# nihofm/volren

Measured on AMD Instinct MI355X. Metric: Msamples/s (pixels x spp / s), volume path tracing, higher is better.
Workload: dtype f32; 1 GPU; BASELINE configs[1] 'c2': smoke.brick, no transfer function, 1024x1024, 1024 spp, seed 42, fov 40; parallelism=1 GPU, 1 fused launch(es)/frame (sample pool budget 64 GiB)

## Files before the change

volren_amd/csrc/capi.cpp:

```cpp
#include "../../include/volren_amd.h"

#include <algorithm>
#include <climits>
#include <cmath>
#include <cstring>
#include <filesystem>
#include <functional>
#include <iostream>
#include <stdexcept>
#include <memory>
#include <string>
#include <vector>

#include "imageio.h"
#include "renderer.h"
#include "sharded.h"
#include "vr_device.h"
#include "vr_math_probe.h"

struct vr_renderer {
    vr::RendererHIP impl;
    int device = 0;
};

struct vr_sharded {
    std::vector<vr_renderer*> parts;
    std::unique_ptr<vr::ShardedRenderer> impl;
    std::string transport, collective;
};

static thread_local std::string g_last_error;

static int guard(const std::function<void()>& fn) {
    try {
        fn();
        g_last_error.clear();
        return VR_OK;
    } catch (const std::exception& e) {
        g_last_error = e.what();
        return VR_ERR;
    } catch (...) {
        g_last_error = "unknown error";
        return VR_ERR;
    }
}
static int fail(int code, const char* msg) { g_last_error = msg; return code; }
#define NEED(r) do { if (!(r)) return fail(VR_ERR_ARG, "null renderer"); } while (0)
#define NEED_SHARDED(s) do { if (!(s)) return fail(VR_ERR_ARG, "null sharded renderer"); } while (0)
#define NEED_DEVICE() do { if (vr_device_count() <= 0) return fail(VR_ERR_NO_DEVICE, "no HIP device available (libvolren_amd has no CPU path)"); } while (0)

static void use_device(vr_renderer* r) { VR_HIP(hipSetDevice(r->device)); }

static int read_back(vr_renderer* r, float* out, void (vr::RendererHIP::*download)(float*)) {
    NEED(r);
    if (!out) return fail(VR_ERR_ARG, "null argument");
    NEED_DEVICE();
    return guard([&] { use_device(r); (r->impl.*download)(out); });
}

namespace {
using Rn = vr::RendererHIP;
struct IntParam {
    const char* name;
    int (*get)(Rn&);
    void (*set)(Rn&, int);
    int lo, hi;
    const char* refusal;
};
vr::SceneParams next_launch(Rn& R) { vr::SceneParams P; R.fill_params(P); return P; }
vr::PathtraceKernel next_kernel(Rn& R) { return vr::pathtrace_kernel_of(next_launch(R), R.tuning.wide_addressing != 0, R.tuning.stats != nullptr); }
void set_grid_frame(Rn& R, int v) {
    if (!R.volume || v < 0 || (size_t)v >= R.volume->n_grid_frames()) throw std::runtime_error("grid_frame_counter out of range");
    R.volume->grid_frame_counter = (size_t)v;
}
#define VR_GET(expr) [](Rn& R) -> int { return expr; }
#define VR_SET(stmt) [](Rn& R, int v) { stmt; }
#define VR_INT(field) VR_GET(R.field), VR_SET(R.field = v)
#define VR_FLAG(field) VR_GET(R.field ? 1 : 0), VR_SET(R.field = v != 0)
#define VR_ANY 1, 0, nullptr
#define VR_READ_ONLY(expr) VR_GET(expr), nullptr, VR_ANY
const IntParam kIntParams[] = {
    { "sample", VR_GET(R.sample), VR_SET(R.sample = v; R.drop_tile_samples()), VR_ANY },
    { "sppx", VR_INT(sppx), VR_ANY },
    { "seed", VR_INT(seed), VR_ANY },
    { "bounces", VR_INT(bounces), VR_ANY },
    { "show_environment", VR_FLAG(show_environment), VR_ANY },
    { "tonemapping", VR_FLAG(tonemapping), VR_ANY },
    { "integrator", VR_INT(integrator), VR_ANY },
    { "fast_math", VR_FLAG(fast_math), VR_ANY },
    { "variance", VR_INT(variance), 0, 1, "variance: 0 (off) or 1 (keep the per-pixel second moments)" },
    { "denoise_iterations", VR_INT(denoise_iterations), 0, vr::kDenoiseMaxIterations, "denoise_iterations must be in [0, 10]" },
    { "denoise_moments", VR_GET(R.denoise_moments), VR_SET(R.set_denoise_moments(v)), VR_ANY },
    { "denoise_resolve", VR_GET(R.denoise_resolve), VR_SET(R.set_denoise_resolve(v)), VR_ANY },
    { "denoise_layers", VR_GET(R.denoise_layers), VR_SET(R.set_denoise_layers(v)), VR_ANY },
    { "denoise_filter", VR_GET(R.denoise_filter), VR_SET(R.set_denoise_filter(v)), VR_ANY },
    { "coalesce_trace", VR_GET(R.coalesce_trace ? 1 : 0), VR_SET(R.flush_pending(); R.coalesce_trace = v != 0), VR_ANY },
    { "majorant_layout", VR_INT(majorant_layout), -1, 1, "majorant_layout: -1 (per grid, chosen at commit), 0 (linear), 1 (4x4x4-cell blocks)" },
    { "majorant_blocked", VR_READ_ONLY(next_launch(R).density.maj_blocked) },
    { "kernel_variant", VR_READ_ONLY(next_kernel(R).variant) },
    { "kernel_variant_reason", VR_READ_ONLY(next_kernel(R).reason) },
    { "tf_float_atlas", VR_FLAG(tf_float_atlas), VR_ANY },
    { "wide_addressing", VR_INT(tuning.wide_addressing), 0, 1, "wide_addressing: 0 (by the tables' sizes), 1 (always the kernels with 64-bit gather addresses)" },
    { "kernel_wide", VR_READ_ONLY(next_kernel(R).wide ? 1 : 0) },
    { "env_div_safe", VR_READ_ONLY(R.environment && R.environment->cdf_div_safe ? 1 : 0) },
    { "env_compact", VR_READ_ONLY(R.environment && R.environment->envmap_rgbe ? 1 : 0) },
    { "pending_samples", VR_READ_ONLY(R.pending_samples()) },
    { "gpu_encoder", VR_FLAG(gpu_encoder), VR_ANY },
    { "sample_pool_mb", VR_GET((int)(R.sample_pool_bytes >> 20)), VR_SET(R.sample_pool_bytes = (size_t)v << 20), 16, 65536,
      "sample_pool_mb must be in [16, 65536] (item indices of a sub-launch are 32-bit: < 2^32 RGBA32F items)" },
    { "seed_table_mb", VR_GET(R.seed_table_budget_mb()), VR_SET(R.seed_table_mb = v), -1, Rn::kSeedTableMaxMb,
      "seed_table_mb must be in [0, 8192] (0 = no table), or -1 for the default min(4096, sample_pool_mb / 4)" },
    { "seed_table_max_samples", VR_INT(seed_table_max_samples), 0, INT_MAX, "seed_table_max_samples must be >= 0 (0 = as many as seed_table_mb holds)" },
    { "seed_table_samples", VR_READ_ONLY(R.seed_table_samples()) },
    { "seed_table_fills", VR_READ_ONLY(R.seed_table_fills()) },
    { "launch_target_ms", VR_INT(launch_target_ms), 0, INT_MAX, "launch_target_ms must be >= 0 (0 = no sizing by time)" },
    { "expected_skip", VR_INT(expected_skip), 0, 1, "expected_skip: 0 (march every step) or 1 (drop the steps of empty space by the clear-distance table)" },
    { "expected_stats", VR_INT(expected_stats), 0, 1, "expected_stats: 0 (off) or 1 (the expected-value passes count their work)" },
    { "order_tiles", VR_INT(order_tiles), 0, 2, "order_tiles: 0 (never), 1 (tile subsets), 2 (always)" },
    { "sky_tiles", VR_INT(sky_tiles), 0, 1, "sky_tiles: 0 (every tile through the path tracer) or 1 (tiles whose camera rays cannot hit the volume's box are rendered apart)" },
    { "last_sky_tiles", VR_READ_ONLY(R.last_sky_tiles) },
    { "grid_frame_counter", VR_GET(R.volume ? (int)R.volume->grid_frame_counter : 0), set_grid_frame, VR_ANY },
    { "n_grid_frames", VR_READ_ONLY(R.volume ? (int)R.volume->n_grid_frames() : 0) },
    { "last_launches", VR_READ_ONLY(R.last_launches) },
    { "adaptive_rounds", VR_READ_ONLY(R.adaptive_rounds) },
    { "width", VR_READ_ONLY(R.resolution.x) },
    { "height", VR_READ_ONLY(R.resolution.y) },
};
#undef VR_GET
#undef VR_SET
#undef VR_INT
#undef VR_FLAG
#undef VR_ANY
#undef VR_READ_ONLY
const IntParam& int_param(const char* name, bool writable) {
    for (const IntParam& p : kIntParams)
        if (!strcmp(p.name, name) && (p.set || !writable)) return p;
    throw std::runtime_error(std::string("unknown int parameter: ") + name);
}

struct FloatField { float* ptr; int count; void (*check)(const float* values, int count) = nullptr; };
FloatField float_field(vr::RendererHIP& R, const std::string& n) {
    if (n == "tonemap_exposure") return { &R.tonemap_exposure, 1 };
    if (n == "tonemap_gamma") return { &R.tonemap_gamma, 1 };
    if (n == "albedo") return { &R.albedo.x, 3 };
    if (n == "phase") return { &R.phase, 1 };
    if (n == "density_scale") return { &R.density_scale, 1 };
    if (n == "emission_scale") return { &R.emission_scale, 1 };
    if (n == "vol_clip_min") return { &R.vol_clip_min.x, 3 };
    if (n == "vol_clip_max") return { &R.vol_clip_max.x, 3 };
    if (n == "cam_pos") return { &R.camera.pos.x, 3 };
    if (n == "cam_dir") return { &R.camera.dir.x, 3 };
    if (n == "cam_up") return { &R.camera.up.x, 3 };
    if (n == "cam_fov") return { &R.camera.fov_degree, 1 };
    if (n == "env_strength") { if (!R.environment) throw std::runtime_error("no environment"); return { &R.environment->strength, 1 }; }
    if (n == "env_transform") { if (!R.environment) throw std::runtime_error("no environment"); return { R.environment->transform.m, 9 }; }
    if (n == "tf_window_left") { if (!R.transferfunc) throw std::runtime_error("no transfer function"); return { &R.transferfunc->window_left, 1 }; }
    if (n == "tf_window_width") { if (!R.transferfunc) throw std::runtime_error("no transfer function"); return { &R.transferfunc->window_width, 1 }; }
    if (n == "volume_transform") { if (!R.volume) throw std::runtime_error("no volume"); return { R.volume->transform.m, 16 }; }
    if (n == "denoise_sigma") return { R.denoise_sigma, 5, [](const float* values, int count) {
        if (count != 5) throw std::runtime_error("denoise_sigma takes 5 values (colour, normal, depth, coverage, albedo)");
        for (int i = 0; i < 5; ++i)
            if (!(values[i] >= vr::kDenoiseSigmaMin && values[i] <= vr::kDenoiseSigmaMax))
                throw std::runtime_error("denoise_sigma: every value must be in [2^-60, 2^60]");
    } };
    if (n == "denoise_alpha") return { &R.denoise_alpha, 1, [](const float* values, int count) {
        if (count == 1 && !(values[0] >= vr::kTemporalAlphaMin && values[0] <= vr::kTemporalAlphaMax)) throw std::runtime_error("denoise_alpha must be in [2^-20, 1]");
    } };
    if (n == "denoise_reject") return { &R.denoise_reject, 1, [](const float* values, int count) {
        if (count == 1 && !(values[0] == 0.0f || (values[0] >= vr::kTemporalRejectMin && values[0] <= vr::kTemporalRejectMax)))
            throw std::runtime_error("denoise_reject must be 0 (off) or in [2^-10, 2^20]");
    } };
    if (n == "denoise_ridge") return { &R.denoise_ridge, 1, [](const float* values, int count) {
        if (count == 1 && !vr::regress_ridge_ok(values[0])) throw std::runtime_error("denoise_ridge must be 0 (zero order) or in [2^-20, 2^20]");
    } };
    throw std::runtime_error("unknown float parameter: " + n);
}
}

extern "C" {

const char* vr_last_error(void) { return g_last_error.c_str(); }
const char* vr_version(void) { return "volren_amd 0.1 (gfx950)"; }

int vr_device_count(void) {
    int n = 0;
    if (hipGetDeviceCount(&n) != hipSuccess) return 0;
    return n;
}

int vr_create(vr_renderer** out, int device, int width, int height) {
    if (!out) return fail(VR_ERR_ARG, "null out pointer");
    *out = nullptr;
    NEED_DEVICE();
    vr_renderer* r = nullptr;
    const int rc = guard([&] {
        if (width <= 0 || height <= 0) throw std::runtime_error("vr_create: resolution must be positive");
        r = new vr_renderer();
        r->device = device;
        use_device(r);
        r->impl.resolution = { width, height };
        r->impl.init();
    });
    if (rc != VR_OK) { delete r; return rc; }
    *out = r;
    return VR_OK;
}

void vr_destroy(vr_renderer* r) {
    if (!r) return;
    (void)hipSetDevice(r->device);
    delete r;
}

int vr_resize(vr_renderer* r, int w, int h) {
    NEED(r);
    return guard([&] { use_device(r); if (w <= 0 || h <= 0) throw std::runtime_error("vr_resize: resolution must be positive"); r->impl.resize((uint32_t)w, (uint32_t)h); r->impl.sample = 0; });
}

int vr_load_volume(vr_renderer* r, const char* path) {
    NEED(r);
    if (!path) return fail(VR_ERR_ARG, "null path");
    return guard([&] {
        use_device(r);
        std::cout << "load volume: " << path << std::endl;
        if (std::filesystem::is_directory(path)) r->impl.volume = vr::Volume::load_folder(path);
        else r->impl.volume = std::make_shared<vr::Volume>(std::string(path));
        r->impl.density_scale = 1.f;
        r->impl.scale_and_move_to_unit_cube();
        r->impl.commit();
        r->impl.sample = 0;
    });
}

int vr_set_volume_path(vr_renderer* r, const char* path) {
    NEED(r);
    if (!path) return fail(VR_ERR_ARG, "null path");
    return guard([&] {
        if (std::filesystem::is_directory(path)) r->impl.volume = vr::Volume::load_folder(path);
        else r->impl.volume = std::make_shared<vr::Volume>(std::string(path));
    });
}

int vr_volume_aabb(vr_renderer* r, const char* name, float out[6]) {
    NEED(r);
    if (!out) return fail(VR_ERR_ARG, "null output");
    return guard([&] {
        if (!r->impl.volume || r->impl.volume->grids.empty()) throw std::runtime_error("vr_volume_aabb: no volume");
        const auto bb = r->impl.volume->AABB(name ? name : "density");
        out[0] = bb.first.x; out[1] = bb.first.y; out[2] = bb.first.z; out[3] = bb.second.x; out[4] = bb.second.y; out[5] = bb.second.z;
    });
}
int vr_volume_minorant_majorant(vr_renderer* r, const char* name, float out[2]) {
    NEED(r);
    if (!out) return fail(VR_ERR_ARG, "null output");
    return guard([&] {
        if (!r->impl.volume || r->impl.volume->grids.empty()) throw std::runtime_error("vr_volume_minorant_majorant: no volume");
        const auto mm = r->impl.volume->minorant_majorant(name ? name : "density");
        out[0] = mm.first; out[1] = mm.second;
    });
}

int vr_load_envmap(vr_renderer* r, const char* path) {
    NEED(r);
    if (!path) return fail(VR_ERR_ARG, "null path");
    return guard([&] { use_device(r); r->impl.environment = std::make_shared<vr::Environment>(std::string(path)); r->impl.sample = 0; });
}

int vr_load_transferfunc(vr_renderer* r, const char* path) {
    NEED(r);
    if (!path) return fail(VR_ERR_ARG, "null path");
    return guard([&] {
        use_device(r);
        r->impl.transferfunc = std::make_shared<vr::TransferFunction>(std::string(path));
// ... 619 lines not shown
```

volren_amd/csrc/renderer.cpp:

```cpp
#include "renderer.h"

#include <algorithm>
#include <cfloat>
#include <cmath>
#include <cstdlib>
#include <cstring>
#include <iostream>
#include <mutex>

#include "vr_adaptive.h"
#include "vr_device.h"
#include "vr_math.h"
#include "vr_path_probe.h"
#include "vr_probe.h"
#include "vr_sky_tiles.h"
#include "vr_upsample.h"

namespace vr {

mat3 Camera::view_inverse() const {
    const vec3 f = normalize(dir);
    const vec3 s = normalize(cross(f, up));
    const vec3 u = cross(s, f);
    mat3 r(0.0f);
    r.m[0] = s.x; r.m[1] = s.y; r.m[2] = s.z;
    r.m[3] = u.x; r.m[4] = u.y; r.m[5] = u.z;
    r.m[6] = -f.x; r.m[7] = -f.y; r.m[8] = -f.z;
    return r;
}

RendererHIP::~RendererHIP() {
    if (ev0_) (void)hipEventDestroy(ev0_);
    if (ev1_) (void)hipEventDestroy(ev1_);
    for (hipEvent_t e : pt_events_) (void)hipEventDestroy(e);
    if (seed_event_) (void)hipEventDestroy(seed_event_);
}

void RendererHIP::init() {
    int n_dev = 0;
    if (hipGetDeviceCount(&n_dev) != hipSuccess || n_dev == 0)
        throw std::runtime_error("RendererHIP::init: no HIP device available (this renderer has no CPU path)");
    if (!volume) volume = std::make_shared<Volume>();
    if (!environment) {
        const float white[3] = { 1.f, 1.f, 1.f };
        environment = std::make_shared<Environment>(white, 1, 1);
    }
    if (!ev0_) { VR_HIP(hipEventCreate(&ev0_)); VR_HIP(hipEventCreate(&ev1_)); }
    if (!status_) {
        status_ = make_device_buffer(16 * sizeof(uint32_t));
        VR_HIP(hipMemset(status_->get(), 0, 16 * sizeof(uint32_t)));
    }
    if (!color && resolution.x > 0 && resolution.y > 0) resize((uint32_t)resolution.x, (uint32_t)resolution.y);
}

void RendererHIP::resize(uint32_t w, uint32_t h) {
    if (w == 0 || h == 0) throw std::runtime_error("RendererHIP::resize: empty framebuffer");
    pending_n_ = 0; pending_ = LaunchInputs{};
    resolution = { (int)w, (int)h };
    color = make_device_buffer((size_t)w * h * 4 * sizeof(float));
    display.reset();
    sized_ = Sized{};
    drop_tile_samples();
    drop_seed_table();
    VR_HIP(hipMemset(color->get(), 0, color->size_bytes()));
    if (!tiles_host_.empty()) set_tiles(tiles_host_);
}

void RendererHIP::reset() { sample = 0; drop_tile_samples(); }

static void check_grid_bytes(size_t bytes, const char* what, const int32_t nb[3]);
constexpr size_t kBlockedMajorantBricks = (size_t)1 << 18;
static size_t brick_records(const BrickGridHIP& g);

void RendererHIP::commit() {
    flush_pending();
    rate_samples_per_ms_ = 0.0; rate_pending_samples_ = 0.0;
    density_grids.clear();
    emission_grids.clear();
    majorant_emission = 0.f;
    maj_key_ = MajKey{};
    std::cout << "Preparing brick grids for HIP..." << std::endl;
    std::vector<size_t> with_emission;
    for (const auto& frame : volume->grids) {
        Volume::GridPtr density_grid = frame.at("density");
        density_grids.push_back(grid_to_device(density_grid));
        Volume::GridPtr emission_grid;
        for (const char* name : { "flame", "flames", "temperature" }) {
            auto it = frame.find(name);
            if (it != frame.end()) { emission_grid = it->second; break; }
        }
        if (emission_grid) {
            emission_grids.push_back(grid_to_device(emission_grid));
            majorant_emission = std::max(majorant_emission, emission_grid->minorant_majorant().second);
            if (emission_grids.size() == density_grids.size()) with_emission.push_back(density_grids.size() - 1);
        }
    }
    for (size_t f : with_emission) {
        BrickGridHIP& gd = density_grids[f];
        BrickGridHIP& ge = emission_grids[f];
        if (!(VR_BRICK_HEADERS && gd.atlas && ge.atlas && grids_can_pair(gd, ge))) continue;
        try {
            const size_t n_rec = brick_records(gd);
            check_grid_bytes(n_rec * kPairBlockBytes, "the paired density + emission atlas", gd.nb);
            auto paired = make_device_buffer(n_rec * kPairBlockBytes);
            launch_pair_atlas(gd.atlas->as<uint8_t>(), ge.atlas->as<uint8_t>(), paired->as<uint8_t>(), n_rec, stream);
            VR_HIP(hipGetLastError());
            VR_HIP(hipStreamSynchronize(stream));
            gd.atlas_paired = ge.atlas_paired = paired;
            gd.maj_blocked = gd.n_active > kBlockedMajorantBricks;
        } catch (const std::exception& e) {
            (void)hipGetLastError();
            std::cerr << "volren_amd: no room for the paired density + emission atlas of frame " << f << " (" << e.what() << "): the run-time kernel variant serves it" << std::endl;
        }
    }
}

BrickGridHIP RendererHIP::grid_to_device(const Volume::GridPtr& grid) {
    if (auto f16 = std::dynamic_pointer_cast<DenseGridF16>(grid)) return dense_grid_to_device(f16);
    if (gpu_encoder)
        if (auto dense = std::dynamic_pointer_cast<DenseGrid>(grid)) return dense_to_bricks_on_device(dense);
    return brick_grid_to_device(Volume::to_brick_grid(grid));
}

static void check_grid_bytes(size_t bytes, const char* what, const int32_t nb[3]) {
    size_t free_b = 0, total_b = 0;
    if (hipMemGetInfo(&free_b, &total_b) != hipSuccess) { (void)hipGetLastError(); return; }
    const size_t reserve = (size_t)1 << 30;
    if (bytes + reserve > free_b)
        throw std::runtime_error(std::string("grid upload: ") + what + " of a grid of " + std::to_string(nb[0]) + " x " + std::to_string(nb[1]) + " x " + std::to_string(nb[2]) +
                                 " bricks needs " + std::to_string(bytes >> 20) + " MiB of device memory, " + std::to_string(free_b >> 20) + " MiB are free");
}
static void set_layout(BrickGridHIP& out) {
    for (int i = 0; i < 3; ++i) out.mshift[i] = std::max(3, ceil_log2((uint32_t)out.nb[i]));
    if (out.mshift[0] + out.mshift[1] + out.mshift[2] > 30 || (uint64_t)out.nb[0] * out.nb[1] * out.nb[2] > 400000000ull)
        throw std::runtime_error("grid upload: more than 4e8 bricks");
    if ((uint64_t)out.nb[1] * out.nb[2] >= (1ull << 24) || out.nb[0] >= (1 << 24))
        throw std::runtime_error("grid upload: brick counts beyond the 24-bit index arithmetic of the kernels (n_bricks.y * n_bricks.z < 2^24)");
    const size_t cells = majorant_table_cells((uint32_t)(out.mshift[0] + out.mshift[1] + out.mshift[2]));
    out.majorant = make_device_buffer(cells * sizeof(float));
    out.majorant16 = make_device_buffer(cells * sizeof(uint16_t));
}
static size_t brick_records(const BrickGridHIP& g) { return (size_t)g.nb[0] * g.nb[1] * g.nb[2]; }

static void upload_range_words(BrickGridHIP& out, const uvec3 nb, const Buf3D<uint32_t>& range, const std::vector<Buf3D<uint32_t>>& mips) {
    if (mips.size() > 3) throw std::runtime_error("grid upload: at most 3 range mips are supported");
    std::vector<uint32_t> words(range.data);
    out.n_mips = (int)mips.size();
    for (int m = 0; m <= 3; ++m) out.mip_off[m] = 0;
    for (int m = 1; m <= out.n_mips; ++m) {
        const auto& mm = mips[m - 1];
        const uint32_t rnd = (1u << m) - 1u;
        if (mm.stride.x != ((nb.x + rnd) >> m) || mm.stride.y != ((nb.y + rnd) >> m) || mm.stride.z != ((nb.z + rnd) >> m))
            throw std::runtime_error("grid upload: range mip dimensions are not ceil(n_bricks / 2^m)");
        out.mip_off[m] = (int32_t)words.size();
        words.insert(words.end(), mm.data.begin(), mm.data.end());
    }
    out.n_cells = (int32_t)words.size();
    out.range_words = make_device_buffer(words.size() * sizeof(uint32_t));
    out.range_words->upload(words.data(), words.size() * sizeof(uint32_t));
    set_layout(out);
}

BrickGridHIP RendererHIP::dense_to_bricks_on_device(const std::shared_ptr<DenseGrid>& g) {
    BrickGridHIP out;
    auto up8 = [](uint32_t v) { return ((v + 7u) / 8u + 7u) / 8u * 8u; };
    const int32_t dim[3] = { (int32_t)g->dim.x, (int32_t)g->dim.y, (int32_t)g->dim.z };
    const int32_t nb[3] = { (int32_t)up8(g->dim.x), (int32_t)up8(g->dim.y), (int32_t)up8(g->dim.z) };
    const size_t n = (size_t)nb[0] * nb[1] * nb[2];
    for (int i = 0; i < 3; ++i) out.nb[i] = nb[i];
    out.transform = g->transform;
    DeviceBuffer dense(g->voxels.size() * sizeof(float)), flag(n * sizeof(uint32_t));
    dense.upload(g->voxels.data(), g->voxels.size() * sizeof(float), stream);
    int32_t mdim[4][3];
    size_t total = 0;
    out.n_mips = 3;
    for (int m = 0; m <= 3; ++m) {
        for (int i = 0; i < 3; ++i) mdim[m][i] = (nb[i] + (1 << m) - 1) >> m;
        out.mip_off[m] = (int32_t)total;
        total += (size_t)mdim[m][0] * mdim[m][1] * mdim[m][2];
    }
    out.n_cells = (int32_t)total;
    out.range_words = make_device_buffer(total * sizeof(uint32_t));
    set_layout(out);
    uint32_t* words = out.range_words->as<uint32_t>();
    launch_encode_ranges(dense.as<float>(), dim, nb, words, flag.as<uint32_t>(), stream);
    VR_HIP(hipGetLastError());
    check_grid_bytes(brick_records(out) * (kBrickBlockBytes + sizeof(BrickRec) + 8), "the brick-linear atlas", out.nb);
    out.atlas = make_device_buffer(brick_records(out) * kBrickBlockBytes);
    VR_HIP(hipMemsetAsync(out.atlas->get(), 0, out.atlas->size_bytes(), stream));
    out.bricks = make_device_buffer(brick_records(out) * sizeof(BrickRec));
    VR_HIP(hipMemsetAsync(out.bricks->get(), 0, out.bricks->size_bytes(), stream));
    out.rng = make_device_buffer(brick_records(out) * 2 * sizeof(float));
    VR_HIP(hipMemsetAsync(out.rng->get(), 0, out.rng->size_bytes(), stream));
    launch_encode_bricks(dense.as<float>(), dim, nb, words, flag.as<uint32_t>(), out.bricks->as<BrickRec>(), out.rng->as<float>(), out.atlas->as<uint8_t>(), stream);
    for (int m = 1; m <= 3; ++m) launch_range_mip(words + out.mip_off[m - 1], mdim[m - 1], words + out.mip_off[m], mdim[m], stream);
    VR_HIP(hipGetLastError());
    VR_HIP(hipStreamSynchronize(stream));
    {
        std::vector<uint32_t> flags(n);
        flag.download(flags.data(), n * sizeof(uint32_t), stream);
        for (uint32_t f : flags) out.n_active += f != 0u;
    }
    return out;
}

constexpr uint64_t kFnv1aStart = 1469598103934665603ull;
static uint64_t fnv1a(const void* p, size_t n, uint64_t h = kFnv1aStart) {
    const uint8_t* b = static_cast<const uint8_t*>(p);
    for (size_t i = 0; i < n; ++i) { h ^= b[i]; h *= 1099511628211ull; }
    return h;
}
void RendererHIP::grid_checksums(const BrickGridHIP& g, uint64_t out[3]) const {
    const DeviceBufferPtr bufs[3] = { g.bricks, g.atlas, g.range_words };
    for (int i = 0; i < 3; ++i) {
        out[i] = 0;
        if (!bufs[i]) continue;
        std::vector<uint8_t> h(bufs[i]->size_bytes());
        bufs[i]->download(h.data(), h.size(), stream);
        out[i] = fnv1a(h.data(), h.size());
    }
}

BrickGridHIP RendererHIP::dense_grid_to_device(const std::shared_ptr<DenseGridF16>& g) {
    BrickGridHIP out;
    const uvec3 nb = g->range.stride;
    out.nb[0] = (int)nb.x; out.nb[1] = (int)nb.y; out.nb[2] = (int)nb.z;
    out.dim[0] = (int)g->dim.x; out.dim[1] = (int)g->dim.y; out.dim[2] = (int)g->dim.z;
    if (g->dim.x > 65535u || g->dim.y > 65535u || g->dim.z > 65535u) throw std::runtime_error("dense_grid_to_device: more than 65535 voxels along an axis");
    out.transform = g->transform;
    const uint32_t bx = (g->dim.x + 3u) / 4u, by = (g->dim.y + 3u) / 4u, bz = (g->dim.z + 3u) / 4u;
    if ((uint64_t)bx * by * bz > (1ull << 31)) throw std::runtime_error("dense_grid_to_device: more than 2^31 blocks");
    out.dblk[0] = (int)bx; out.dblk[1] = (int)by;
    std::vector<uint16_t> blocked((size_t)bx * by * bz * 64u, 0);
    for (uint32_t z = 0; z < g->dim.z; ++z)
        for (uint32_t y = 0; y < g->dim.y; ++y) {
            const uint16_t* row = &g->voxels[((size_t)z * g->dim.y + y) * g->dim.x];
            for (uint32_t x = 0; x < g->dim.x; ++x) blocked[dense_blocked_index(x, y, z, bx, by)] = row[x];
        }
// ... 74 lines not shown
    v.bricks = g.bricks ? g.bricks->as<BrickRec>() : nullptr;
    v.atlas = paired ? g.atlas_paired->as<uint8_t>() : (g.atlas ? g.atlas->as<uint8_t>() : nullptr);
    v.dense = g.dense ? g.dense->as<uint16_t>() : nullptr;
    for (int i = 0; i < 3; ++i) v.dim[i] = g.dim[i];
    for (int i = 0; i < 2; ++i) v.dblk[i] = g.dblk[i];
    v.majorant = g.majorant->as<float>();
    v.majorant16 = g.majorant16->as<uint16_t>();
    v.rng = g.rng ? g.rng->as<float>() : nullptr;
    v.atlas_f32 = g.atlas_f32 ? g.atlas_f32->as<float>() : nullptr;
    for (int i = 0; i < 3; ++i) v.nb[i] = g.nb[i];
    for (int i = 0; i < 3; ++i) { v.mshift[i] = g.mshift[i]; v.mlim[i] = (float)(8u << g.mshift[i]); }
    v.n_mips = g.n_mips;
    v.maj_blocked = maj_blocked ? 1 : 0;
    v.maj_outside = (int32_t)majorant_padded_cells((uint32_t)(g.mshift[0] + g.mshift[1] + g.mshift[2]));
    return v;
}

void RendererHIP::fill_params(SceneParams& P) {
    if (!volume || volume->grids.empty() || density_grids.empty())
        throw std::runtime_error("RendererHIP::trace: no volume committed");
    if (volume->grid_frame_counter >= density_grids.size())
        throw std::runtime_error("RendererHIP::trace: grid_frame_counter out of range (commit() after changing the volume)");
    memset(&P, 0, sizeof P);
    Uniforms& u = P.u;
    u.bounces = bounces;
    u.seed = seed;
    u.show_environment = show_environment ? 1 : 0;
    u.integrator = integrator;
    P.env_div_safe = environment->cdf_div_safe ? 1 : 0;
    copy3(u.cam_pos, camera.pos);
    u.cam_fov = camera.fov_degree;
    const mat3 ct = camera.view_inverse();
    memcpy(u.cam_transform, ct.m, sizeof ct.m);
    P.cam_z = camera_z(camera.fov_degree);
    const auto [bb_min, bb_max] = volume->AABB();
    const auto [mn, maj] = volume->minorant_majorant();
    copy3(u.vol_bb_min, bb_min + vol_clip_min * (bb_max - bb_min));
    copy3(u.vol_bb_max, bb_min + vol_clip_max * (bb_max - bb_min));
    u.vol_minorant = mn * density_scale;
    u.vol_majorant = maj * density_scale;
    u.vol_inv_majorant = 1.f / (maj * density_scale);
    copy3(u.vol_albedo, albedo);
    u.vol_phase_g = phase;
    u.vol_density_scale = density_scale;
    u.vol_emission_scale = emission_scale;
    u.vol_emission_norm = majorant_emission > 0.f ? 1.f / std::fmax(majorant_emission, 1e-4f) : 1.f;
    const BrickGridHIP& density = density_grids[volume->grid_frame_counter];
    const mat4 dt = volume->transform * density.transform;
    const mat4 dti = inverse(dt);
    memcpy(u.vol_density_transform, dt.m, sizeof dt.m);
    memcpy(u.vol_density_inv_transform, dti.m, sizeof dti.m);
    P.density = make_view(density);
    if (volume->grid_frame_counter < emission_grids.size()) {
        const BrickGridHIP& emission = emission_grids[volume->grid_frame_counter];
        const mat4 et = volume->transform * emission.transform;
        const mat4 eti = inverse(et);
        memcpy(u.vol_emission_transform, et.m, sizeof et.m);
        memcpy(u.vol_emission_inv_transform, eti.m, sizeof eti.m);
        const mat4 efd = eti * dt;
        memcpy(P.emission_from_density, efd.m, sizeof efd.m);
        P.paired = (density.atlas_paired && density.atlas_paired == emission.atlas_paired && pathtrace_scene_reasons(P) == 0) ? 1 : 0;
        if (P.paired) P.density = make_view(density, true, majorant_layout < 0 ? density.maj_blocked : majorant_layout == 1);
        P.emission = make_view(emission, P.paired != 0);
        u.has_emission = 1;
    }
    if (transferfunc) {
        u.use_tf = 1;
        u.tf_size = transferfunc->size();
        u.tf_window_left = transferfunc->window_left;
        u.tf_window_width = transferfunc->window_width;
        P.tf_lut = transferfunc->lut_ssbo->as<float>();
    }
    const mat3 eit = inverse(environment->transform);
    memcpy(u.env_transform, environment->transform.m, sizeof eit.m);
    memcpy(u.env_inv_transform, eit.m, sizeof eit.m);
    u.env_strength = environment->strength;
    u.env_imp_inv_dim[0] = u.env_imp_inv_dim[1] = 1.f / (float)environment->dimension();
    u.env_imp_base_mip = (int)std::floor(std::log2((float)environment->dimension()));
    P.envmap = environment->envmap->as<float>();
    P.env_rgbe = environment->envmap_rgbe ? environment->envmap_rgbe->as<uint32_t>() : nullptr;
    P.env_w = environment->width; P.env_h = environment->height;
    P.env_avg_w = environment->avg_importance; P.env_avg_w_set = 1;
    P.impmap = environment->impmap->as<float>();
    P.imp_dim = (int)environment->dimension();
    P.env_cdf = environment->cdf->as<float>();
    u.resolution[0] = resolution.x; u.resolution[1] = resolution.y;
}

void RendererHIP::update_majorants(const LaunchInputs& in, BrickGridHIP& g) {
    if (in.maj == maj_key_) return;
    launch_majorants(in.P, g.range_words->as<uint32_t>(), g.nb, g.mip_off, g.n_mips, g.mshift, g.majorant->as<float>(), g.majorant16->as<uint16_t>(), in.stream);
    VR_HIP(hipGetLastError());
    maj_key_ = in.maj;
}

void RendererHIP::set_tiles(const std::vector<int32_t>& tile_ids) {
    flush_pending();
    tiles_host_ = tile_ids;
    tiles_dev_.reset();
    if (tile_ids.empty()) return;
    if (resolution.x > 0) {
        const int n_all = tile_count(resolution.x, resolution.y);
        for (int32_t t : tile_ids)
            if (t < 0 || t >= n_all) throw std::runtime_error("set_tiles: tile id out of range");
    }
    tiles_dev_ = make_device_buffer(tile_ids.size() * sizeof(int32_t));
    tiles_dev_->upload(tile_ids.data(), tile_ids.size() * sizeof(int32_t));
}

std::vector<int32_t> RendererHIP::costliest_first(const SceneParams& P, const std::vector<int32_t>& tile_ids, int n_tiles) const {
    const Uniforms& u = P.u;
    const int W = u.resolution[0], H = u.resolution[1], tiles_x = vr::tiles_x(W);
    std::vector<int32_t> ids(tile_ids);
    if (ids.empty()) { ids.resize((size_t)n_tiles); for (int i = 0; i < n_tiles; ++i) ids[(size_t)i] = i; }
    auto chord = [&](float px, float py) {
        float d[3] = { (px - 0.5f * (float)W) / (float)H, (py - 0.5f * (float)H) / (float)H, P.cam_z };
        float w[3];
        for (int i = 0; i < 3; ++i) w[i] = u.cam_transform[i] * d[0] + u.cam_transform[3 + i] * d[1] + u.cam_transform[6 + i] * d[2];
        const float len = std::sqrt(w[0] * w[0] + w[1] * w[1] + w[2] * w[2]);
        float t0 = 0.f, t1 = FLT_MAX;
        for (int i = 0; i < 3; ++i) {
            const float inv = 1.f / (w[i] / len);
            const float a = (u.vol_bb_min[i] - u.cam_pos[i]) * inv, b = (u.vol_bb_max[i] - u.cam_pos[i]) * inv;
            t0 = std::fmax(t0, std::fmin(a, b)); t1 = std::fmin(t1, std::fmax(a, b));
        }
        return t1 > t0 ? t1 - t0 : 0.f;
    };
    std::vector<float> cost(ids.size());
    for (size_t k = 0; k < ids.size(); ++k) {
        const float x0 = (float)((ids[k] % tiles_x) * 16), y0 = (float)((ids[k] / tiles_x) * 16);
        const float x1 = std::fmin(x0 + 16.f, (float)W), y1 = std::fmin(y0 + 16.f, (float)H);
        cost[k] = std::fmax(std::fmax(std::fmax(chord(x0, y0), chord(x1, y0)), std::fmax(chord(x0, y1), chord(x1, y1))), chord(0.5f * (x0 + x1), 0.5f * (y0 + y1)));
    }
    std::vector<int32_t> perm(ids.size());
    for (size_t k = 0; k < perm.size(); ++k) perm[k] = (int32_t)k;
    const size_t seg = (ids.size() + 7) / 8;
    for (size_t b = 0; b < ids.size(); b += seg)
        std::stable_sort(perm.begin() + (ptrdiff_t)b, perm.begin() + (ptrdiff_t)std::min(ids.size(), b + seg), [&](int32_t x, int32_t y) { return cost[(size_t)x] > cost[(size_t)y]; });
    std::vector<int32_t> ordered(ids.size());
    for (size_t k = 0; k < ids.size(); ++k) ordered[k] = ids[(size_t)perm[k]];
    return ordered;
}

uint64_t RendererHIP::tile_order_key(const SceneParams& P, const std::vector<int32_t>& ids, int n_tiles) const {
    const Uniforms& u = P.u;
    uint64_t key = kFnv1aStart;
    auto mix = [&key](const void* p, size_t nbytes) { key = fnv1a(p, nbytes, key); };
    mix(u.cam_pos, sizeof u.cam_pos); mix(u.cam_transform, sizeof u.cam_transform); mix(&P.cam_z, sizeof P.cam_z);
    mix(u.vol_bb_min, sizeof u.vol_bb_min); mix(u.vol_bb_max, sizeof u.vol_bb_max); mix(u.resolution, sizeof u.resolution); mix(&n_tiles, sizeof n_tiles);
    if (!ids.empty()) mix(ids.data(), ids.size() * sizeof(int32_t));
    return key ? key : 1;
}

RendererHIP::SplitTiles RendererHIP::split_tiles(const SceneParams& P, const std::vector<int32_t>& ids, int n_tiles, bool ordered) {
    const int tag = ordered ? 2 : 1;
    uint64_t key = fnv1a(&tag, sizeof tag, tile_order_key(P, ids, n_tiles));
    key = key ? key : 1;
    if (split_key_ != key) {
        std::vector<int32_t> march, sky;
        sky_split_tiles(P, ids, n_tiles, march, sky);
        if (!sky.empty()) {
            if (ordered && !march.empty()) march = costliest_first(P, march, (int)march.size());
            march.insert(march.end(), sky.begin(), sky.end());
            ensure_buffer(split_dev_, march.size() * sizeof(int32_t));
            split_dev_->upload(march.data(), march.size() * sizeof(int32_t), stream);
        }
        split_n_sky_ = (int)sky.size();
        split_key_ = key;
    }
    SplitTiles s;
    if (split_n_sky_ > 0) {
        s.n_sky = split_n_sky_;
        s.n_march = n_tiles - split_n_sky_;
        s.march = split_dev_->as<int32_t>();
        s.sky = s.march + s.n_march;
    }
    return s;
}

const int32_t* RendererHIP::tile_order(const SceneParams& P, const std::vector<int32_t>& ids, int n_tiles) {
    const uint64_t key = tile_order_key(P, ids, n_tiles);
    if (order_dev_ && order_key_ == key && order_dev_->size_bytes() == (size_t)n_tiles * sizeof(int32_t)) return order_dev_->as<int32_t>();
    const std::vector<int32_t> ordered = costliest_first(P, ids, n_tiles);
    ensure_buffer(order_dev_, ordered.size() * sizeof(int32_t));
    order_dev_->upload(ordered.data(), ordered.size() * sizeof(int32_t), stream);
    order_key_ = key;
    return order_dev_->as<int32_t>();
}

bool RendererHIP::LaunchInputs::same_launch_as(const LaunchInputs& o) const {
    return memcmp(&P, &o.P, sizeof P) == 0 && frame == o.frame && maj == o.maj && tuning == o.tuning && order_tiles == o.order_tiles && launch_target_ms == o.launch_target_ms &&
           fast_math == o.fast_math && variance == o.variance && sky_tiles == o.sky_tiles && sample_pool_bytes == o.sample_pool_bytes && stream == o.stream;
}

void RendererHIP::capture(LaunchInputs& in) {
    if (!color) throw std::runtime_error("RendererHIP::trace: no framebuffer (call resize first)");
    if (integrator == 2 && !transferfunc) throw std::runtime_error("RendererHIP::trace: integrator 2 (direct volume rendering) needs a transfer function");
    if (integrator < 0 || integrator > 3) throw std::runtime_error("RendererHIP::trace: unknown integrator");
    if (fast_math && transferfunc) throw std::runtime_error("RendererHIP::trace: fast_math is not available while a transfer function is bound (it misses the 1e-3 bound there); set fast_math 0");
    if (!volume || volume->grids.empty() || density_grids.empty()) throw std::runtime_error("RendererHIP::trace: no volume committed");
    if (volume->grid_frame_counter >= density_grids.size()) throw std::runtime_error("RendererHIP::trace: grid_frame_counter out of range (commit() after changing the volume)");
    {
        BrickGridHIP& g = density_grids[volume->grid_frame_counter];
        const bool build = transferfunc && tf_float_atlas && !g.dense && g.atlas && g.rng && !g.atlas_f32 && !g.atlas_f32_failed;
        const bool drop = (!transferfunc || !tf_float_atlas) && (g.atlas_f32 || g.atlas_f32_failed);
        if (build || drop) flush_pending();
        if (build) {
            try {
                const size_t n_blocks = g.atlas->size_bytes() / kBrickBlockBytes, want = n_blocks * 512u * sizeof(float);
                auto drop_others = [&] { for (BrickGridHIP& other : density_grids) if (&other != &g) other.atlas_f32.reset(); };
                size_t free_b = 0, total_b = 0;
                if (hipMemGetInfo(&free_b, &total_b) != hipSuccess) { (void)hipGetLastError(); free_b = ~(size_t)0; }
                if (want > free_b / 2) drop_others();
                try { g.atlas_f32 = make_device_buffer(want); }
                catch (const std::exception&) { (void)hipGetLastError(); drop_others(); g.atlas_f32 = make_device_buffer(want); }
                launch_decode_atlas(g.rng->as<float>(), g.atlas->as<uint8_t>(), g.atlas_f32->as<float>(), n_blocks, stream);
                VR_HIP(hipGetLastError());
            } catch (const std::exception& e) {
                (void)hipGetLastError();
                g.atlas_f32.reset();
                g.atlas_f32_failed = true;
                std::cerr << "volren_amd: no room for the decoded float atlas (" << (g.atlas->size_bytes() / kBrickBlockBytes * 2048u >> 20) << " MiB): transfer-function taps read the byte atlas (" << e.what() << ")" << std::endl;
            }
        }
        if (drop) { g.atlas_f32.reset(); g.atlas_f32_failed = false; }
    }
    fill_params(in.P);
    in.frame = volume->grid_frame_counter;
    in.maj = MajKey{};
    in.maj.density_scale = density_scale;
    in.maj.tf_version = transferfunc ? transferfunc->version : 0;
    in.maj.wl = transferfunc ? transferfunc->window_left : 0.f;
    in.maj.ww = transferfunc ? transferfunc->window_width : 0.f;
    in.maj.frame = in.frame;
    in.maj.blocked = in.P.density.maj_blocked;
    in.tuning = tuning;
    in.order_tiles = order_tiles; in.launch_target_ms = launch_target_ms; in.fast_math = fast_math ? 1 : 0; in.variance = variance != 0 ? 1 : 0; in.sky_tiles = sky_tiles != 0 ? 1 : 0;
    in.sample_pool_bytes = sample_pool_bytes;
    in.stream = stream;
    in.env = environment; in.tf = transferfunc;
    in.keep[0] = environment->envmap; in.keep[1] = environment->impmap; in.keep[2] = environment->cdf;
    in.keep[3] = transferfunc ? transferfunc->lut_ssbo : DeviceBufferPtr();
    in.keep[4] = environment->envmap_rgbe;
}

int RendererHIP::samples_per_launch(const LaunchInputs& in, int n_tiles) const {
    const size_t per_sample = pathtrace_pool_floats(in.tuning, n_tiles, 1) * sizeof(float);
    int per_launch = (int)std::max<size_t>(1, in.sample_pool_bytes / per_sample);
    const size_t lim = (size_t)0xFFFFFFFFu / ((size_t)n_tiles * 256u);
    per_launch = (int)std::min<size_t>((size_t)per_launch, lim > 8 ? lim - 8 : 1);
    if (per_launch > 32) per_launch -= per_launch % 32;
    return per_launch;
}

void RendererHIP::submit_tile_set(const LaunchInputs& in, int first, int n) {
    if (n <= 0) return;
    const int n_tiles = tile_set_size();
    const bool ordered = in.order_tiles >= 2 || (in.order_tiles == 1 && tiles_dev_);
    const SplitTiles split = in.splits_sky() ? split_tiles(in.P, tiles_dev_ ? tiles_host_ : std::vector<int32_t>(), n_tiles, ordered) : SplitTiles{};
    if (split.n_sky > 0) {
        const int per_launch = prepare_submit(in, first, n, split.n_march, split.n_sky);
        open_timing_window(in.stream);
        submit(in, first, n, split.march, split.n_march, per_launch, split.sky, split.n_sky);
        close_timing_window(in.stream);
        return;
    }
    const int32_t* tiles = ordered ? tile_order(in.P, tiles_host_, n_tiles) : (tiles_dev_ ? tiles_dev_->as<int32_t>() : nullptr);
    const int per_launch = prepare_submit(in, first, n, n_tiles);
    open_timing_window(in.stream);
    submit(in, first, n, tiles, n_tiles, per_launch);
    close_timing_window(in.stream);
}

int RendererHIP::tile_set_size() const { return tiles_dev_ ? (int)tiles_host_.size() : tile_count(resolution.x, resolution.y); }

void RendererHIP::open_timing_window(hipStream_t s) { VR_HIP(hipEventRecord(ev0_, s)); last_launches = 0; pt_events_used_ = 0; }
void RendererHIP::close_timing_window(hipStream_t s) { VR_HIP(hipEventRecord(ev1_, s)); timing_pending_ = true; }

int RendererHIP::prepare_submit(const LaunchInputs& in, int first, int n, int n_tiles, int n_sky) {
    if (n <= 0) return 0;
    hipStream_t stream = in.stream;
    update_majorants(in, density_grids.at(in.frame));
    int per_launch = n_tiles > 0 ? std::min(samples_per_launch(in, n_tiles + n_sky), n) : n;
    for (; n_tiles > 0;) {
        const size_t need = pathtrace_pool_floats(in.tuning, n_tiles, per_launch) * sizeof(float);
        if (pool_ && pool_->size_bytes() >= need) break;
        if (pool_) { VR_HIP(hipStreamSynchronize(stream)); pool_.reset(); }
        try { pool_ = make_device_buffer(need); break; }
        catch (const std::exception&) {
            (void)hipGetLastError();
            if (per_launch <= 1) throw;
            per_launch = std::max(1, per_launch / 2);
            if (per_launch > 32) per_launch -= per_launch % 32;
        }
    }
    if (!workspace_ && n_tiles > 0) {
        workspace_ = make_device_buffer(pathtrace_workspace_floats() * sizeof(float));
        if (const char* e = std::getenv("VR_TEST_POISON_WORKSPACE"); e && *e == '1') VR_HIP(hipMemsetAsync(workspace_->get(), 0xFF, workspace_->size_bytes(), stream));
    }
    if (const char* e = std::getenv("VR_TEST_POISON_WORKSPACE"); e && *e == '2' && n_tiles > 0) {
        VR_HIP(hipMemsetAsync(workspace_->get(), 0xFF, workspace_->size_bytes(), stream));
        VR_HIP(hipMemsetAsync(pool_->get(), 0xFF, pool_->size_bytes(), stream));
    }
    if (in.launch_target_ms > 0 && in.kernel().item_integrator == 0) harvest_rate(false);
    if (in.variance && ensure_buffer(sized_.moments, color->size_bytes())) {
        VR_HIP(hipMemsetAsync(sized_.moments->get(), 0, color->size_bytes(), stream));
        if (first > 0) sized_.moments_n = -1;
    }
    sized_.moments_n = !in.variance ? -1 : (first == 0 ? n : (sized_.moments_n == first ? first + n : -1));
    return per_launch;
}

void RendererHIP::submit(const LaunchInputs& in, int first, int n, const int32_t* tiles, int n_tiles, int per_launch, const int32_t* sky, int n_sky) {
    const SceneParams& P = in.P;
    last_sky_tiles = n_sky;
    hipStream_t stream = in.stream;
    const PathtraceKernel kernel = in.kernel();
    const bool pt_kernel = kernel.item_integrator == 0;
    const double px_samples = (double)(n_tiles + n_sky) * 256.0;
    const uint64_t key = [&] {
        uint64_t h = kFnv1aStart;
        auto mix = [&h](const void* p, size_t nbytes) { h = fnv1a(p, nbytes, h); };
        const Uniforms& u = P.u;
        mix(&u.bounces, sizeof u.bounces); mix(u.vol_albedo, sizeof u.vol_albedo); mix(&u.vol_phase_g, sizeof u.vol_phase_g); mix(&u.vol_density_scale, sizeof u.vol_density_scale);
        mix(&u.use_tf, sizeof u.use_tf); mix(&u.tf_window_left, sizeof u.tf_window_left); mix(&u.tf_window_width, sizeof u.tf_window_width); mix(&u.integrator, sizeof u.integrator);
        mix(&u.has_emission, sizeof u.has_emission); mix(u.resolution, sizeof u.resolution); mix(u.vol_bb_min, sizeof u.vol_bb_min); mix(u.vol_bb_max, sizeof u.vol_bb_max);
        const size_t frame = in.frame; mix(&frame, sizeof frame); mix(&n_tiles, sizeof n_tiles);
        const uint64_t tfv = in.maj.tf_version; mix(&tfv, sizeof tfv);
        return h ? h : 1ull;
    }();
    auto cap_by_rate = [&](int planned) {
        if (in.launch_target_ms <= 0 || rate_samples_per_ms_ <= 0.0) return planned;
        const double cap = rate_samples_per_ms_ * (double)in.launch_target_ms / px_samples;
        int c = cap >= (double)planned ? planned : std::max(1, (int)cap);
        if (c > 32) c -= c % 32;
        return c;
    };
    int probe = 0;
    if (pt_kernel && in.launch_target_ms > 0) {
        const bool known = rate_samples_per_ms_ > 0.0 && rate_key_ == key;
        if (!known && px_samples * (double)std::min(per_launch, n) > (double)(1u << 26)) {
            rate_samples_per_ms_ = 0.0;
            probe = (int)std::min<double>(32.0, std::max(1.0, (double)(1u << 24) / px_samples));
            probe = std::min(probe, n);
        } else per_launch = cap_by_rate(per_launch);
    }
    float* moments = in.variance ? sized_.moments->as<float>() : nullptr;
    for (int done = 0; done < n;) {
        if (n_tiles > 0) ++last_launches;
        const int m = probe > 0 ? probe : std::min(per_launch, n - done);
        hipEvent_t eb = nullptr, ee = nullptr;
        if (pt_kernel) {
            while (pt_events_.size() < pt_events_used_ + 2) { hipEvent_t e; VR_HIP(hipEventCreate(&e)); pt_events_.push_back(e); }
            eb = pt_events_[pt_events_used_]; ee = pt_events_[pt_events_used_ + 1];
            pt_events_used_ += 2;
        }
        int seed_samples = 0;
        const uint32_t* seed_table = kernel.reads_seed_table ? seed_table_for(P, first + done, m, stream, &seed_samples) : nullptr;
        launch_pathtrace(in.tuning, P, color->as<float>(), n_tiles > 0 ? pool_->as<float>() : nullptr, n_tiles > 0 ? workspace_->as<float>() : nullptr, status_->as<uint32_t>() + 1, tiles, n_tiles, first + 1 + done, m,
                         status_->as<uint32_t>(), stream, in.fast_math != 0, eb, ee, moments, seed_table, seed_samples, sky, n_sky);
        VR_HIP(hipGetLastError());
        done += m;
        if (pt_kernel) { rate_pending_samples_ = px_samples * (double)m; rate_pending_key_ = key; }
        if (probe > 0) {
            probe = 0;
            harvest_rate(true);
            per_launch = cap_by_rate(per_launch);
        }
    }
}

int RendererHIP::seed_table_samples_for(long long mb, int w, int h) {
    if (mb <= 0 || w <= 0 || h <= 0) return 0;
    const long long per_sample = (long long)tile_count(w, h) * 256 * (long long)sizeof(uint32_t);
    return (int)std::min<long long>((mb << 20) / per_sample, 1 << 24);
}

void RendererHIP::drop_seed_table() {
    seed_table_.reset();
    seed_cap_ = seed_filled_ = 0;
    seed_failed_ = false;
}

const uint32_t* RendererHIP::seed_table_for(const SceneParams& P, int s0, int n, hipStream_t stream, int* samples) {
    *samples = 0;
    const int W = P.u.resolution[0], H = P.u.resolution[1], budget_mb = seed_table_budget_mb();
    if (seed_key_[0] != P.u.seed || seed_key_[1] != W || seed_key_[2] != H || seed_budget_mb_ != budget_mb || seed_max_samples_ != seed_table_max_samples) {
        drop_seed_table();
        seed_key_[0] = P.u.seed; seed_key_[1] = W; seed_key_[2] = H; seed_budget_mb_ = budget_mb; seed_max_samples_ = seed_table_max_samples;
    }
    int max_samples = seed_table_samples_for(budget_mb, W, H);
    if (seed_table_max_samples > 0) max_samples = std::min(max_samples, seed_table_max_samples);
    if (max_samples <= 0 || (seed_failed_ && !seed_table_) || s0 < 0 || n <= 0) return nullptr;
    const size_t per_sample = (size_t)tile_count(W, H) * 256u * sizeof(uint32_t);
    const int want = (int)std::min<long long>((long long)s0 + n, max_samples);
    if (!seed_event_) VR_HIP(hipEventCreateWithFlags(&seed_event_, hipEventDisableTiming));
    if (seed_table_ && seed_filled_ > 0 && stream != seed_stream_) { VR_HIP(hipStreamWaitEvent(stream, seed_event_, 0)); seed_stream_ = stream; }
    if (want > seed_cap_ && !seed_failed_) {
        const int cap = (int)std::min<long long>(max_samples, std::max<long long>(want, 2ll * seed_cap_));
        DeviceBufferPtr grown;
        try { grown = make_device_buffer((size_t)cap * per_sample); }
        catch (const std::exception& e) {
            (void)hipGetLastError();
            seed_failed_ = true;
            static std::once_flag once;
            std::call_once(once, [&] { fprintf(stderr, "volren_amd: note: no memory for the path-seed table (%zu MiB: %s); new paths hash their seeds (slower; results unchanged)\n", ((size_t)cap * per_sample) >> 20, e.what()); });
            if (!seed_table_) return nullptr;
        }
        if (grown) {
            if (const char* e = std::getenv("VR_TEST_POISON_WORKSPACE"); e && *e == '2') VR_HIP(hipMemsetAsync(grown->get(), 0xFF, grown->size_bytes(), stream));
            if (seed_filled_ > 0) VR_HIP(hipMemcpyAsync(grown->get(), seed_table_->get(), (size_t)seed_filled_ * per_sample, hipMemcpyDeviceToDevice, stream));
            if (seed_table_) VR_HIP(hipStreamSynchronize(stream));
            seed_table_ = grown;
            seed_cap_ = cap;
        }
    }
    const int upto = std::min(want, seed_cap_);
    if (upto > seed_filled_) {
        launch_seed_fill(seed_table_->as<uint32_t>(), (uint32_t)P.u.seed, W, H, seed_filled_, upto, stream);
        VR_HIP(hipGetLastError());
        VR_HIP(hipEventRecord(seed_event_, stream));
        seed_stream_ = stream;
        seed_filled_ = upto;
        ++seed_fills_;
    }
    *samples = seed_filled_;
    return seed_filled_ > 0 ? seed_table_->as<uint32_t>() : nullptr;
}

void RendererHIP::harvest_rate(bool wait) {
    if (rate_pending_samples_ <= 0.0 || pt_events_used_ < 2) return;
    hipEvent_t eb = pt_events_[pt_events_used_ - 2], ee = pt_events_[pt_events_used_ - 1];
    if (wait) VR_HIP(hipEventSynchronize(ee));
    else if (hipEventQuery(ee) != hipSuccess) { (void)hipGetLastError(); return; }
    float ms = 0.f;
    if (hipEventElapsedTime(&ms, eb, ee) != hipSuccess || !(ms > 0.f)) { (void)hipGetLastError(); return; }
    rate_samples_per_ms_ = rate_pending_samples_ / (double)ms;
    rate_key_ = rate_pending_key_;
    rate_pending_samples_ = 0.0;
}

void RendererHIP::trace() {
    if (ragged())
        throw std::runtime_error("trace: the frame holds per-tile sample counts of render_adaptive (a ragged frame): reset(), or continue with render_adaptive");
    if (!coalesce_trace) { flush_pending(); LaunchInputs in; capture(in); submit_tile_set(in, sample, 1); sample += 1; return; }
    LaunchInputs now;
    capture(now);
    if (pending_n_ > 0 && (sample != pending_first_ + pending_n_ || !now.same_launch_as(pending_))) flush_pending();
    if (pending_n_ == 0) {
        pending_ = std::move(now);
        pending_first_ = sample;
        pending_cap_ = samples_per_launch(pending_, tile_set_size());
    }
    ++pending_n_;
    ++sample;
    if (pending_n_ >= pending_cap_) flush_pending();
}

void RendererHIP::flush_pending() {
    if (pending_n_ <= 0) return;
    const int n = pending_n_, first = pending_first_;
    pending_n_ = 0;
    LaunchInputs in = std::move(pending_);
    pending_ = LaunchInputs{};
    submit_tile_set(in, first, n);
}

void RendererHIP::render(int n) {
    flush_pending();
    if (ragged()) throw std::runtime_error("render: the frame holds per-tile sample counts of render_adaptive (a ragged frame): reset(), or continue with render_adaptive");
    if (n <= 0) n = sppx - sample;
    if (n <= 0) return;
    LaunchInputs in;
    capture(in);
    submit_tile_set(in, sample, n);
    sample += n;
}

void RendererHIP::draw() {
    flush_pending();
    if (!color) return;
    draw_from(*color);
}

void RendererHIP::draw_from(const DeviceBuffer& src) {
    ensure_buffer(display, src.size_bytes());
    VR_HIP(hipMemcpyAsync(display->get(), src.get(), src.size_bytes(), hipMemcpyDeviceToDevice, stream));
    if (tonemapping) {
        launch_tonemap(display->as<float>(), (int32_t)(src.size_bytes() / (4 * sizeof(float))), 1, tonemap_exposure, tonemap_gamma, stream);
        VR_HIP(hipGetLastError());
    }
}

double RendererHIP::last_kernel_ms() {
    flush_pending();
    if (timing_pending_) {
        VR_HIP(hipEventSynchronize(ev1_));
        float ms = 0.f;
        VR_HIP(hipEventElapsedTime(&ms, ev0_, ev1_));
        last_ms_ = (double)ms;
        last_pathtrace_ms_ = 0.0;
        for (size_t i = 0; i + 1 < pt_events_used_; i += 2)
            if (hipEventElapsedTime(&ms, pt_events_[i], pt_events_[i + 1]) == hipSuccess) last_pathtrace_ms_ += (double)ms;
        (void)hipGetLastError();
        timing_pending_ = false;
    }
    return last_ms_;
}

double RendererHIP::last_pathtrace_ms() { (void)last_kernel_ms(); return last_pathtrace_ms_; }

void RendererHIP::sched_stats(bool enable, unsigned long long out[32]) {
    flush_pending();
// ... 443 lines not shown
        throw std::runtime_error(me + "the expected-value pass ran with rays = " + std::to_string(sized_.rays) + "; rays >= 2 is needed (one ray gives the coverage of the pixel's centre, not of its area)");
    if ((size_t)resolution.x * (size_t)resolution.y * 2u > (size_t)INT32_MAX) throw std::runtime_error(me + "frame too large (32-bit pixel indices)");
}

void RendererHIP::run_resolve() {
    LaunchInputs in;
    capture(in);
    const size_t bytes = (size_t)resolution.x * resolution.y * 4 * sizeof(float);
    ensure_buffer(sized_.rs_bg, bytes); ensure_buffer(sized_.rs_part, bytes); ensure_buffer(sized_.resolved, bytes);
    launch_resolve(in.P, color->as<float>(), sized_.features->as<float>(), sized_.rays, sized_.rs_bg->as<float>(), sized_.rs_part->as<float>(), sized_.resolved->as<float>(), stream);
    VR_HIP(hipGetLastError());
}

void RendererHIP::resolve() {
    flush_pending();
    check_resolve("resolve: ", false);
    run_resolve();
}

void RendererHIP::download_resolved(float* rgba) { download_whole(sized_.resolved, rgba, "resolved: no resolve since the last resize (call resolve first)"); }

void RendererHIP::download_resolve_background(float* rgba) {
    download_whole(sized_.resolved ? sized_.rs_bg : nullptr, rgba, "resolve_background: no resolve since the last resize (call resolve first)");
}

void RendererHIP::download_denoised_layer(float* rgba) {
    download_whole(sized_.layer_valid ? sized_.layer : nullptr, rgba, "denoised_layer: no denoise with denoise_layers = 1 since the last resize");
}

void RendererHIP::upsample(int factor, int rays) {
    if (factor < kUpsampleMinFactor || factor > kUpsampleMaxFactor) throw std::runtime_error("upsample: factor must be 2..4");
    if (rays < 1 || rays > kExpectedMaxRays) throw std::runtime_error("upsample: rays must be 1.." + std::to_string(kExpectedMaxRays));
    flush_pending();
    if (!sized_.layer_valid) throw std::runtime_error("upsample: no denoise with denoise_layers = 1 since the last resize (its layer is what the call upsamples)");
    if (!sized_.layer_guided)
        throw std::runtime_error("upsample: the last denoise ran with denoise_layers = 0 and its guide has replaced the layer's (denoise with denoise_layers = 1 again; denoised_layer stays readable)");
    if (!tiles_host_.empty() && !sized_.layer_gathered) throw std::runtime_error("upsample: a tile subset is set (set_tiles); the call rebuilds whole frames only");
    const int32_t w = resolution.x, h = resolution.y, W = factor * w, H = factor * h;
    const size_t px = (size_t)W * (size_t)H;
    if (px * 2u > (size_t)INT32_MAX) throw std::runtime_error("upsample: the upsampled frame is too large (32-bit pixel indices)");
    SceneParams P;
    feature_scene(P);
    P.u.resolution[0] = W; P.u.resolution[1] = H;
    if (sized_.up_factor != factor) { sized_.up_factor = 0; sized_.up_features.reset(); sized_.up_out.reset(); sized_.up_layer.reset(); }
    ensure_buffer(sized_.up_features, px * 8 * sizeof(float));
    ensure_buffer(sized_.up_out, px * 4 * sizeof(float));
    ensure_buffer(sized_.up_layer, px * 4 * sizeof(float));
    launch_expected(P, nullptr, tile_count(W, H), rays, sized_.up_features->as<float>());
    const DenoiseSigma sg = sigma();
    launch_upsample(P, sized_.layer->as<float>(), sized_.dn_guide->as<float>(), w, h, factor, sized_.up_features->as<float>(), rays, sg, sized_.up_out->as<float>(),
                    sized_.up_layer->as<float>(), stream);
    VR_HIP(hipGetLastError());
    sized_.up_factor = factor;
}

static const char* const kNoUpsample = "upsampled: no upsample since the last resize (call upsample first)";
void RendererHIP::download_upsampled(float* rgba) { download_whole(sized_.up_factor ? sized_.up_out : nullptr, rgba, kNoUpsample); }
void RendererHIP::download_upsampled_layer(float* rgba) { download_whole(sized_.up_factor ? sized_.up_layer : nullptr, rgba, kNoUpsample); }
void RendererHIP::download_upsampled_features(float* out) { download_whole(sized_.up_factor ? sized_.up_features : nullptr, out, kNoUpsample); }
void RendererHIP::upsampled_size(int wh[2]) const {
    if (!sized_.up_factor) throw std::runtime_error(kNoUpsample);
    wh[0] = sized_.up_factor * resolution.x; wh[1] = sized_.up_factor * resolution.y;
}

void RendererHIP::download_history_moments(float* out) {
    const Sized::History& hist = sized_.hist;
    download_whole(hist.cur < 0 ? nullptr : hist.moments[hist.cur], out,
                   "denoise_history_moments: no history with moment records (no denoise_temporal with denoise_moments = 1 since the last resize, history reset or change of the setting)");
}

void RendererHIP::download_history(float* rgba, float* var, float* length) {
    const Sized::History& hist = sized_.hist;
    if (hist.cur < 0) throw std::runtime_error("denoise_history: no history (no denoise_temporal since the last resize or history reset)");
    flush_pending();
    if (rgba) hist.color[hist.cur]->download(rgba, hist.color[hist.cur]->size_bytes(), stream);
    if (!var && !length) return;
    const size_t px = (size_t)resolution.x * resolution.y;
    std::vector<float> rec(px * 4);
    hist.record[hist.cur]->download(rec.data(), rec.size() * sizeof(float), stream);
    for (size_t i = 0; i < px; ++i) {
        if (var) var[i] = rec[4 * i];
        if (length) length[i] = rec[4 * i + 1];
    }
}

void RendererHIP::download_reject_stat(float* out) {
    if (!sized_.reject_stat) throw std::runtime_error("denoise_reject_stat: the last denoise_temporal since the resize did not run with denoise_reject > 0");
    flush_pending();
    const size_t px = (size_t)resolution.x * resolution.y;
    std::vector<float> rec(px * 4);
    VR_HIP(hipMemcpyAsync(rec.data(), sized_.dn_reject->as<float>() + px * 4, rec.size() * sizeof(float), hipMemcpyDeviceToHost, stream));
    VR_HIP(hipStreamSynchronize(stream));
    for (size_t i = 0; i < px; ++i) out[i] = rec[4 * i];
}

void RendererHIP::download_denoised(float* rgba) { download_whole(sized_.denoised, rgba, "denoised: no denoise since the last resize (call denoise first)"); }

bool RendererHIP::ragged() {
    if (!tile_n_.empty() && sample != tile_n_sample_) drop_tile_samples();
    return !tile_n_.empty();
}

void RendererHIP::drop_tile_samples() { tile_n_.clear(); tile_n_sample_ = -1; }

std::vector<int32_t> RendererHIP::tile_samples() {
    flush_pending();
    if (ragged()) return tile_n_;
    return std::vector<int32_t>((size_t)tile_count(resolution.x, resolution.y), sample);
}

std::vector<float> RendererHIP::tile_error() {
    flush_pending();
    if (!color) throw std::runtime_error("tile_error: no framebuffer");
    check_moments("tile_error");
    const std::vector<int32_t> counts = tile_samples();
    const int n_all = (int)counts.size();
    std::vector<int32_t> lists((size_t)n_all * 2);
    for (int t = 0; t < n_all; ++t) { lists[(size_t)t] = t; lists[(size_t)(n_all + t)] = counts[(size_t)t]; }
    ensure_buffer_at_least(sized_.adaptive_lists, lists.size() * sizeof(int32_t));
    ensure_buffer_at_least(sized_.adaptive_err, (size_t)n_all * sizeof(float));
    sized_.adaptive_lists->upload(lists.data(), lists.size() * sizeof(int32_t), stream);
    launch_adaptive_error(color->as<float>(), sized_.moments->as<float>(), sized_.adaptive_lists->as<int32_t>(), sized_.adaptive_lists->as<int32_t>() + n_all, n_all, resolution.x,
                          resolution.y, sized_.adaptive_err->as<float>(), stream);
    VR_HIP(hipGetLastError());
    std::vector<float> e((size_t)n_all);
    sized_.adaptive_err->download(e.data(), e.size() * sizeof(float), stream);
    return e;
}

void RendererHIP::render_adaptive(int min_spp, int max_spp, float threshold) {
    if (min_spp < 2 || min_spp > max_spp || !(threshold >= 0.0f) || !std::isfinite(threshold))
        throw std::invalid_argument("render_adaptive: needs 2 <= min_spp <= max_spp and a finite threshold >= 0");
    flush_pending();
    if (!color) throw std::runtime_error("render_adaptive: no framebuffer (call resize first)");
    const bool was_ragged = ragged();
    if (sample > 0 && !was_ragged && !(sized_.moments && sized_.moments_n == sample))
        throw std::runtime_error("render_adaptive: the moments do not cover samples 1.." + std::to_string(sample) +
                                 " (variance was off for some of them): reset() and render with variance = 1");
    LaunchInputs in;
    capture(in);
    in.variance = 1;
    const int W = resolution.x, H = resolution.y, n_all = tile_count(W, H);
    if (!was_ragged) tile_n_.assign((size_t)n_all, std::max(sample, 0));
    std::vector<int32_t> set(tiles_host_);
    if (set.empty()) { set.resize((size_t)n_all); for (int t = 0; t < n_all; ++t) set[(size_t)t] = t; }
    ensure_buffer_at_least(sized_.adaptive_lists, (size_t)n_all * 2 * sizeof(int32_t));
    ensure_buffer_at_least(sized_.adaptive_err, (size_t)n_all * sizeof(float));
    const bool ordered = in.order_tiles >= 1, split = in.splits_sky();
    open_timing_window(in.stream);
    adaptive_rounds = 0;
    auto launch_groups = [&](const std::vector<int32_t>& ids, const auto& to) {
        const auto groups = adaptive_groups(ids, tile_n_);
        std::vector<int32_t> packed;
        std::vector<int> n_sky;
        for (const auto& g : groups) {
            std::vector<int32_t> march = g.second, sky;
            if (split) sky_split_tiles(in.P, g.second, (int)g.second.size(), march, sky);
            if (ordered && !march.empty()) march = costliest_first(in.P, march, (int)march.size());
            packed.insert(packed.end(), march.begin(), march.end());
            packed.insert(packed.end(), sky.begin(), sky.end());
            n_sky.push_back((int)sky.size());
        }
        if (packed.empty()) return;
        sized_.adaptive_lists->upload(packed.data(), packed.size() * sizeof(int32_t), in.stream);
        size_t off = 0, k = 0;
        for (const auto& g : groups) {
            const int32_t n = g.first, next = to(n);
            const int n_clear = n_sky[k++], n_tiles = (int)g.second.size() - n_clear;
            const int32_t* list = sized_.adaptive_lists->as<int32_t>() + off;
            submit(in, n, next - n, list, n_tiles, prepare_submit(in, n, next - n, n_tiles, n_clear), n_clear > 0 ? list + n_tiles : nullptr, n_clear);
            for (int32_t t : g.second) tile_n_[(size_t)t] = next;
            off += g.second.size();
        }
    };
    auto finish = [&] {
        close_timing_window(in.stream);
        const auto mm = std::minmax_element(tile_n_.begin(), tile_n_.end());
        sample = *mm.second;
        if (*mm.first == *mm.second) { drop_tile_samples(); sized_.moments_n = sample; }
        else { tile_n_sample_ = sample; sized_.moments_n = -1; }
    };
    try {
        std::vector<int32_t> low;
        for (int32_t t : set) if (tile_n_[(size_t)t] < min_spp) low.push_back(t);
        launch_groups(low, [&](int32_t) { return min_spp; });
        std::vector<int32_t> live, go;
        for (int32_t t : set) if (tile_n_[(size_t)t] < max_spp) live.push_back(t);
        while (!live.empty()) {
            ++adaptive_rounds;
            const size_t m = live.size();
            std::vector<int32_t> lists(live);
            for (int32_t t : live) lists.push_back(tile_n_[(size_t)t]);
            sized_.adaptive_lists->upload(lists.data(), lists.size() * sizeof(int32_t), in.stream);
            launch_adaptive_error(color->as<float>(), sized_.moments->as<float>(), sized_.adaptive_lists->as<int32_t>(), sized_.adaptive_lists->as<int32_t>() + m, (int32_t)m, W, H,
                                  sized_.adaptive_err->as<float>(), in.stream);
            VR_HIP(hipGetLastError());
            std::vector<float> e(m);
            sized_.adaptive_err->download(e.data(), m * sizeof(float), in.stream);
            check_watchdog();
            go.clear();
            for (size_t k = 0; k < m; ++k) if (!adaptive_converged(e[k], threshold)) go.push_back(live[k]);
            launch_groups(go, [&](int32_t n) { return adaptive_next_count(n, max_spp); });
            live.clear();
            for (int32_t t : go) if (tile_n_[(size_t)t] < max_spp) live.push_back(t);
        }
    } catch (...) {
        finish();
        throw;
    }
    finish();
}

void RendererHIP::check_watchdog() {
    const uint32_t st = watchdog_status();
    if (st & kSkyHitStatus) throw std::runtime_error("sky tiles: a camera ray of a tile classified clear hit the volume's box (vr_sky_tiles.h sky_tile_clear is wrong for this view); the pixels concerned stopped at that sample. Render with sky_tiles 0");
    if (st & kFeatureLostStatus) throw std::runtime_error("feature pass: a camera segment exceeded its step budget (vr_render_features); the pixels concerned cover only their samples before it");
    if (st != 0) throw std::runtime_error("path-tracing kernel watchdog tripped (a wavefront exceeded its step budget)");
}

uint32_t RendererHIP::watchdog_status() {
    flush_pending();
    uint32_t s = 0;
    status_->download(&s, sizeof s, stream);
    if (s != 0) {
        VR_HIP(hipMemsetAsync(status_->get(), 0, sizeof(uint32_t), stream));
        VR_HIP(hipStreamSynchronize(stream));
    }
    return s;
}

}
```

volren_amd/csrc/renderer.h:

```cpp
#pragma once

#include <algorithm>
#include <memory>
#include <string>
#include <vector>

#include "devmem.h"
#include "environment.h"
#include "grids.h"
#include "transferfunc.h"
#include "vr_device.h"
#include "vr_regress.h"
#include "vr_scene.h"

namespace vr {

struct Camera {
    vec3 pos{ 1.f, 0.f, 1.f };
    vec3 dir = normalize(-pos);
    vec3 up{ 0.f, 1.f, 0.f };
    float fov_degree = 70.f;
    mat3 view_inverse() const;
};

struct BrickGridHIP {
    DeviceBufferPtr bricks;
    DeviceBufferPtr atlas;
    DeviceBufferPtr range_words;
    DeviceBufferPtr majorant;
    DeviceBufferPtr majorant16;
    DeviceBufferPtr rng;
    DeviceBufferPtr atlas_f32;
    bool atlas_f32_failed = false;
    DeviceBufferPtr atlas_paired;
    DeviceBufferPtr clear_table;
    DeviceBufferPtr dense;
    int32_t dim[3] = { 0, 0, 0 };
    int32_t dblk[2] = { 0, 0 };
    int32_t nb[3] = { 0, 0, 0 };
    int32_t mip_off[4] = { 0, 0, 0, 0 };
    int32_t n_mips = 0;
    int32_t n_cells = 0;
    int32_t mshift[3] = { 3, 3, 3 };
    size_t n_active = 0;
    bool maj_blocked = false;
    mat4 transform;
};

struct RendererHIP {
    void init();
    void resize(uint32_t w, uint32_t h);
    void commit();
    void trace();
    void draw();
    void reset();

    void render(int n = 0);
    void render_adaptive(int min_spp, int max_spp, float threshold);
    std::vector<int32_t> tile_samples();
    std::vector<float> tile_error();
    bool ragged();
    void drop_tile_samples();
    void check_watchdog();

    BrickGridHIP brick_grid_to_device(const std::shared_ptr<BrickGrid>& grid);
    BrickGridHIP dense_grid_to_device(const std::shared_ptr<DenseGridF16>& grid);
    BrickGridHIP grid_to_device(const Volume::GridPtr& grid);
    BrickGridHIP dense_to_bricks_on_device(const std::shared_ptr<DenseGrid>& grid);
    bool gpu_encoder = true;
    void grid_checksums(const BrickGridHIP& g, uint64_t out[3]) const;
    void scale_and_move_to_unit_cube();

    int sample = 0;
    int sppx = 1024;
    int seed = 42;
    int bounces = 100;
    float tonemap_exposure = 5.f;
    float tonemap_gamma = 2.2f;
    bool tonemapping = true;
    bool show_environment = true;

    vec3 albedo = vec3(0.9f);
    float phase = 0.f;
    float density_scale = 1.f;
    float emission_scale = 100.f;

    DeviceBufferPtr color;
    DeviceBufferPtr display;
    std::vector<BrickGridHIP> density_grids;
    std::vector<BrickGridHIP> emission_grids;
    float majorant_emission = 0.f;

    std::shared_ptr<Volume> volume;

    vec3 vol_clip_min = vec3(0.f);
    vec3 vol_clip_max = vec3(1.f);

    std::shared_ptr<Environment> environment;
    std::shared_ptr<TransferFunction> transferfunc;

    Camera camera;
    ivec2 resolution{ 0, 0 };
    hipStream_t stream = nullptr;
    int integrator = 0;
    bool tf_float_atlas = true;
    int order_tiles = 1;
    int majorant_layout = -1;
    int variance = 0;
    int denoise_iterations = kDenoiseDefaultIterations;
    float denoise_sigma[5] = { kDenoiseDefaultSigma[0], kDenoiseDefaultSigma[1], kDenoiseDefaultSigma[2], kDenoiseDefaultSigma[3], kDenoiseDefaultSigma[4] };
    float denoise_alpha = kTemporalDefaultAlpha;
    int denoise_moments = 0;
    float denoise_reject = 0.0f;
    bool fast_math = false;
    PathtraceTuning tuning = default_tuning();
    int sky_tiles = 1;
    int last_sky_tiles = 0;
    int last_launches = 0;
    int adaptive_rounds = 0;
    int launch_target_ms = 2000;
    size_t sample_pool_bytes = (size_t)64 << 30;

    int seed_table_mb = -1;
    int seed_table_max_samples = 0;
    static constexpr int kSeedTableMaxMb = 8192;
    static int seed_table_default_mb(long long sample_pool_mb) { return (int)std::min<long long>(4096, sample_pool_mb / 4); }
    static int seed_table_samples_for(long long mb, int w, int h);
    int seed_table_budget_mb() const { return seed_table_mb >= 0 ? seed_table_mb : seed_table_default_mb((long long)(sample_pool_bytes >> 20)); }
    int seed_table_samples() const { return seed_filled_; }
    int seed_table_fills() const { return seed_fills_; }
    void set_tiles(const std::vector<int32_t>& tile_ids);
    void fill_params(SceneParams& P);
    void download(float* rgba);
    void render_features(int spp);
    void render_features_expected(int rays);
    int expected_skip = 1;
    int expected_stats = 0;
    void expected_stats_read(uint64_t out[4]);
    void expected_clear_table(uint8_t* out, int cells[3]);
    void probe(int what, int form, const uint32_t* in, float* out, size_t n);
    void path_probe(int kind, int form, const uint32_t* in, uint32_t* out, size_t n);
    void filter_probe(int stage, int W, int H, const void* const* in, float* const* out, const float* params);
    void download_features(float* out);
    void download_variance(float* rgba);
    void denoise();
    void denoise_temporal();
    void drop_history();
    void resolve();
    void check_resolve(const std::string& me, bool whole_frame_gathered);
    void download_resolved(float* rgba);
    void download_resolve_background(float* rgba);
    void set_denoise_resolve(int v);
    int denoise_resolve = 0;
    void set_denoise_layers(int v);
    int denoise_layers = 0;
    void download_denoised_layer(float* rgba);
    void set_denoise_filter(int v);
    int denoise_filter = 0;
    void set_denoise_ridge(float v);
    float denoise_ridge = kRegressDefaultRidge;
    void upsample(int factor, int rays);
    void download_upsampled(float* rgba);
    void download_upsampled_layer(float* rgba);
    void download_upsampled_features(float* out);
    void upsampled_size(int wh[2]) const;
    const DeviceBuffer* upsampled() const { return sized_.up_factor ? sized_.up_out.get() : nullptr; }
    void download_history(float* rgba, float* var, float* length);
    void download_reject_stat(float* out);
    void set_denoise_moments(int v);
    void download_history_moments(float* out);
    void download_denoised(float* rgba);
    const DeviceBuffer* denoised() const { return sized_.denoised.get(); }
    const DeviceBuffer* resolved() const { return sized_.resolved.get(); }
    void draw_from(const DeviceBuffer& src);
    void download_display(float* rgba) const;
    void synchronize();
    void flush_pending();
    int begin_feature_pass(SceneParams& P);
    void feature_scene(SceneParams& P);
    void launch_expected(const SceneParams& P, const int32_t* tiles, int n_tiles, int rays, float* out);
    int pending_samples() const { return pending_n_; }
    bool coalesce_trace = true;
    double last_kernel_ms();
    double last_pathtrace_ms();
    void sched_stats(bool enable, unsigned long long out[32]);
    void wave_timeline(unsigned long long* out, size_t n_words);
    uint32_t watchdog_status();
    ~RendererHIP();

private:
    struct MajKey {
        float density_scale = -1.f; uint64_t tf_version = ~0ull; float wl = 0, ww = 0; size_t frame = ~(size_t)0; int blocked = -1;
        bool operator==(const MajKey& o) const { return density_scale == o.density_scale && tf_version == o.tf_version && wl == o.wl && ww == o.ww && frame == o.frame && blocked == o.blocked; }
    };
    struct LaunchInputs {
        SceneParams P;
        MajKey maj;
        size_t frame = 0;
        PathtraceTuning tuning;
        int order_tiles = 0, launch_target_ms = 0, fast_math = 0, variance = 0, sky_tiles = 0;
        size_t sample_pool_bytes = 0;
        hipStream_t stream = nullptr;
        std::shared_ptr<Environment> env;
        std::shared_ptr<TransferFunction> tf;
        DeviceBufferPtr keep[5];
        bool same_launch_as(const LaunchInputs& o) const;
        PathtraceKernel kernel() const { return pathtrace_kernel_of(P, tuning.wide_addressing != 0, tuning.stats != nullptr); }
        bool splits_sky() const { return sky_tiles != 0 && tuning.stats == nullptr && fast_math == 0 && kernel().item_integrator == 0; }
    };
    void capture(LaunchInputs& in);
    int prepare_submit(const LaunchInputs& in, int first, int n, int n_tiles, int n_sky = 0);
    void submit(const LaunchInputs& in, int first, int n, const int32_t* tiles, int n_tiles, int per_launch, const int32_t* sky = nullptr, int n_sky = 0);
    void submit_tile_set(const LaunchInputs& in, int first, int n);
    void open_timing_window(hipStream_t s), close_timing_window(hipStream_t s);
    int tile_set_size() const;
    void unpair_views(SceneParams& P, size_t frame) const;
    int samples_per_launch(const LaunchInputs& in, int n_tiles) const;
    LaunchInputs pending_;
    int pending_n_ = 0, pending_first_ = 0, pending_cap_ = 0;
    void update_majorants(const LaunchInputs& in, BrickGridHIP& g);
    std::vector<int32_t> tiles_host_;
    DeviceBufferPtr tiles_dev_;
    DeviceBufferPtr order_dev_;
    uint64_t order_key_ = 0;
    std::vector<int32_t> costliest_first(const SceneParams& P, const std::vector<int32_t>& ids, int n_tiles) const;
    const int32_t* tile_order(const SceneParams& P, const std::vector<int32_t>& ids, int n_tiles);
    uint64_t tile_order_key(const SceneParams& P, const std::vector<int32_t>& ids, int n_tiles) const;
    struct SplitTiles { const int32_t* march = nullptr; int n_march = 0; const int32_t* sky = nullptr; int n_sky = 0; };
    SplitTiles split_tiles(const SceneParams& P, const std::vector<int32_t>& ids, int n_tiles, bool ordered);
    DeviceBufferPtr split_dev_;
    uint64_t split_key_ = 0;
    int split_n_sky_ = 0;
    std::vector<int32_t> tile_n_;
    int tile_n_sample_ = -1;
    DeviceBufferPtr status_;
    DeviceBufferPtr pool_;
    DeviceBufferPtr workspace_;
    DeviceBufferPtr seed_table_;
    int seed_cap_ = 0, seed_filled_ = 0, seed_fills_ = 0, seed_budget_mb_ = -1, seed_max_samples_ = 0;
    int seed_key_[3] = { 0, 0, 0 };
    bool seed_failed_ = false;
    hipStream_t seed_stream_ = nullptr;
    hipEvent_t seed_event_ = nullptr;
    void drop_seed_table();
    const uint32_t* seed_table_for(const SceneParams& P, int s0, int n, hipStream_t stream, int* samples);
    DeviceBufferPtr stats_;
    struct Sized {
        DeviceBufferPtr features;
        int pass = 0, rays = 0;
        DeviceBufferPtr moments;
        int moments_n = -1;
        DeviceBufferPtr rs_bg, rs_part, resolved;
        DeviceBufferPtr ly_split, ly_filtered, layer;
        bool layer_valid = false;
        bool layer_guided = false;
        bool layer_gathered = false;
        DeviceBufferPtr up_features, up_out, up_layer;
        int up_factor = 0;
        DeviceBufferPtr dn_guide, dn_var[2], dn_color[2];
        DeviceBufferPtr denoised;
        DeviceBufferPtr dn_reject;
        bool reject_stat = false;
        DeviceBufferPtr tile_n_dev, adaptive_lists, adaptive_err;
        struct History {
            DeviceBufferPtr color[2], record[2];
            DeviceBufferPtr moments[2];
            int cur = -1;
            bool layers = false;
            TemporalCamera cam{};
        } hist;
    } sized_;
    void download_whole(const DeviceBufferPtr& b, float* out, const char* absent);
    void run_resolve();
    void set_history_switch(int& field, int v, const char* refusal);
    DenoiseSigma sigma() const { return { denoise_sigma[0], denoise_sigma[1], denoise_sigma[2], denoise_sigma[3], denoise_sigma[4] }; }
    DeviceBufferPtr expected_stats_;
    bool expected_stats_valid_ = false;
    ClearTable clear_table_of(BrickGridHIP& g, const GridView& view);
    void check_moments(const char* who);
    void run_denoise(const char* who, bool temporal, bool whole_frame_gathered = false);
    friend struct ShardedRenderer;
    hipEvent_t ev0_ = nullptr, ev1_ = nullptr;
    std::vector<hipEvent_t> pt_events_;
    size_t pt_events_used_ = 0;
    double last_ms_ = 0.0, last_pathtrace_ms_ = 0.0;
    bool timing_pending_ = false;
    double rate_samples_per_ms_ = 0.0;
    uint64_t rate_key_ = 0, rate_pending_key_ = 0;
    double rate_pending_samples_ = 0.0;
    void harvest_rate(bool wait);
    MajKey maj_key_;
};

using Renderer = RendererHIP;

}
```

volren_amd/csrc/vr_device.h:

```cpp
#pragma once

#include <hip/hip_runtime.h>
#include <stdint.h>

#include "vr_denoise.h"
#include "vr_scene.h"
#include "vr_temporal.h"
#include "vr_tiles.h"
#include "vr_variant.h"

namespace vr {

struct PathtraceTuning {
    int32_t thr[8] = { 64, 0, 56, 0, 60, 60, 64, 0 };
    unsigned long long* stats = nullptr;
    int32_t samples_per_unit = 0;
    int32_t blocks_per_cu = 0;
    int32_t wide_addressing = 0;
    bool operator==(const PathtraceTuning& o) const {
        for (int i = 0; i < 8; ++i) if (thr[i] != o.thr[i]) return false;
        return stats == o.stats && samples_per_unit == o.samples_per_unit && blocks_per_cu == o.blocks_per_cu && wide_addressing == o.wide_addressing;
    }
};
PathtraceTuning default_tuning();
size_t pathtrace_pool_floats(const PathtraceTuning& T, int32_t n_tiles, int32_t n_samples);
size_t pathtrace_workspace_floats();
void launch_pathtrace(const PathtraceTuning& T, const SceneParams& P, float* fb, float* sample_pool, float* workspace, uint32_t* unit_counter, const int32_t* tiles, int32_t n_tiles,
                      int32_t first_sample, int32_t n_samples, uint32_t* status, hipStream_t stream, bool fast_math = false,
                      hipEvent_t ev_kernel_begin = nullptr, hipEvent_t ev_kernel_end = nullptr,
                      float* moments = nullptr,
                      const uint32_t* seed_table = nullptr, int32_t seed_samples = 0,
                      const int32_t* sky_tiles = nullptr, int32_t n_sky_tiles = 0);
constexpr uint32_t kSkyHitStatus = 8u;
constexpr uint32_t kFeatureLostStatus = 4u;
void launch_features(const SceneParams& P, const int32_t* tiles, int32_t n_tiles, int32_t spp, float* out, uint32_t* status, hipStream_t stream);
constexpr int32_t kExpectedMaxRays = 4;
void launch_features_expected(const SceneParams& P, const int32_t* tiles, int32_t n_tiles, int32_t rays, float* out, hipStream_t stream,
                              const ClearTable* clear = nullptr, unsigned long long* stats = nullptr);
void launch_denoise_prepare(const float* moments, const float* features, int32_t W, int32_t H, int32_t n, float vscale, const int32_t* counts, float* v, float* guide,
                            hipStream_t stream);
void launch_denoise_atrous(const float* cin, const float* vin, const float* guide, int32_t W, int32_t H, int32_t step, const DenoiseSigma& sg,
                           float* cout, float* vout, hipStream_t stream);
struct TemporalPass {
    const float* color = nullptr;
    float* v = nullptr;
    const float* guide = nullptr;
    const float *hist_color = nullptr, *hist_record = nullptr, *hist_moments = nullptr;
    bool same_cam = false;
    TemporalCamera cur{}, prev{};
    int32_t W = 0, H = 0;
    float alpha = 1.0f;
    float tau = 0.0f;
    float* scratch = nullptr;
    DenoiseSigma sigma{};
    float *out_color = nullptr, *out_record = nullptr, *out_moments = nullptr;
};
void launch_denoise_temporal(const TemporalPass& t, hipStream_t stream);
void launch_resolve(const SceneParams& P, const float* fb, const float* features, int32_t rays, float* B, float* Pq, float* out, hipStream_t stream);
void launch_layers_split(const float* y, const float* B, const float* features, int32_t W, int32_t H, float* S, hipStream_t stream);
void launch_layers_merge(const float* F, const float* B, const float* features, int32_t W, int32_t H, float* out, float* L, hipStream_t stream);
void launch_denoise_regress(const float* S, const float* guide, int32_t W, int32_t H, const DenoiseSigma& sg, float ridge, float* F, hipStream_t stream);
void launch_upsample(const SceneParams& P, const float* lo_layer, const float* lo_guide, int32_t w, int32_t h, int32_t f, const float* hi_features, int32_t rays,
                     const DenoiseSigma& sg, float* out, float* L, hipStream_t stream);
void launch_adaptive_error(const float* fb, const float* moments, const int32_t* tiles, const int32_t* counts, int32_t n_tiles, int32_t W, int32_t H, float* out,
                           hipStream_t stream);

void launch_tonemap(float* fb, int32_t w, int32_t h, float exposure, float gamma, hipStream_t stream);

void launch_pack_tiles(const float* fb, int32_t w, int32_t h, const int32_t* tiles, int32_t n_tiles, float* packed, hipStream_t stream);
void launch_unpack_tiles(const float* packed, const int32_t* tiles, int32_t n_tiles, float* fb, int32_t w, int32_t h, hipStream_t stream);
void launch_pack_guides(const float* moments, const float* features, int32_t w, int32_t h, const int32_t* tiles, int32_t n_tiles, float* packed, hipStream_t stream);
void launch_unpack_guides(const float* packed, const int32_t* tiles, int32_t n_tiles, float* moments, float* features, int32_t w, int32_t h, hipStream_t stream);
void launch_build_impmap(const float* envmap_rgba, int32_t env_w, int32_t env_h, int32_t dim, float* pyramid, hipStream_t stream);

void launch_build_env_cdf(const float* pyramid, int32_t dim, float* table, uint32_t* unsafe_flag, hipStream_t stream);

void launch_majorants(const SceneParams& P, const uint32_t* range_words_all_mips, const int32_t nb[3], const int32_t mip_off[4], int32_t n_mips,
                      const int32_t mshift[3], float* out_padded, uint16_t* out16_padded, hipStream_t stream);

void launch_encode_ranges(const float* dense, const int32_t dim[3], const int32_t nb[3], uint32_t* range, uint32_t* flag, hipStream_t stream);
void launch_encode_bricks(const float* dense, const int32_t dim[3], const int32_t nb[3], const uint32_t* range, const uint32_t* flag,
                          BrickRec* recs, float* rng, uint8_t* atlas, hipStream_t stream);
void launch_range_mip(const uint32_t* src, const int32_t sdim[3], uint32_t* dst, const int32_t ddim[3], hipStream_t stream);

void launch_pair_atlas(const uint8_t* atlas_density, const uint8_t* atlas_emission, uint8_t* out, size_t n_records, hipStream_t stream);

void launch_decode_atlas(const float* rng, const uint8_t* atlas, float* out, size_t n_records, hipStream_t stream);
void launch_clear_table(const GridView& g, uint8_t* table, uint8_t* scratch, hipStream_t stream);
void launch_seed_fill(uint32_t* table, uint32_t seed, int32_t W, int32_t H, int32_t s_begin, int32_t s_end, hipStream_t stream);
void launch_math_probe(int32_t fn, const float* a, const float* b, float* out, int32_t n, hipStream_t stream);
void launch_math_sweep(int32_t fn, uint32_t first, float b, float* out, int32_t n, hipStream_t stream);
void launch_fast_math_sweep(int32_t fn, uint32_t first, float* out, int32_t n, hipStream_t stream);
void launch_probe(const SceneParams& P, int32_t what, int32_t form, const uint32_t* in, float* out, uint32_t n, hipStream_t stream);
void launch_path_probe(const SceneParams& P, int32_t kind, int32_t form, const uint32_t* in, uint32_t* out, uint32_t n, hipStream_t stream);

}
```

volren_amd/csrc/vr_launch.hip:

```cpp
#include <hip/hip_runtime.h>

#include <algorithm>
#include <cstdlib>
#include <map>
#include <mutex>
#include <stdexcept>
#include <string>

#include "vr_device.h"
#include "vr_expected.h"
#include "vr_pathtrace.h"

namespace vr {

template <int INTEGRATOR>
__global__ void __launch_bounds__(256)
item_kernel(const SceneParams P, float* __restrict__ sbuf, const LaunchDesc D) {
    const uint32_t per_unit = (uint32_t)(D.spu * 64);
    const uint32_t g = blockIdx.x * 256u + threadIdx.x;
    const uint32_t u = g / per_unit, item = g - u * per_unit;
    if (u >= D.n_units) return;
    const WorkUnit wu = make_unit(D, P.u.resolution[0], u, sbuf);
    if ((int32_t)item >= wu.n_items) return;
    const int32_t px = wu.px0 + (int32_t)(item & 7u), py = wu.py0 + (int32_t)((item >> 3) & 7u);
    if (px >= P.u.resolution[0] || py >= P.u.resolution[1]) return;
    float L[4];
    if (INTEGRATOR == 2) dvr_sample(P, px, py, wu.first_sample + (int32_t)(item >> 6), L);
    else raymarch_path_sample(P, px, py, wu.first_sample + (int32_t)(item >> 6), L);
    reinterpret_cast<float4*>(sbuf)[wu.base + item] = pack4(L);
}

template <bool MOMENTS>
__device__ __forceinline__ void fold_sample(float acc[4], float S[4], const float L[4], int32_t current_sample) {
    const float a = 1.0f / (float)current_sample;
    for (int32_t c = 0; c < 4; ++c) {
        const float x = sanitize(L[c]);
        const float mu = acc[c], mu1 = mix_(mu, x, a);
        if (MOMENTS) S[c] = mix_(S[c], (x - mu) * (x - mu1), a);
        acc[c] = mu1;
    }
}

template <bool MOMENTS>
__global__ void __launch_bounds__(256)
accumulate_kernel(const float* __restrict__ sbuf, float* __restrict__ fb, float* __restrict__ moments, const int32_t* __restrict__ tiles, int32_t n_tiles,
                  int32_t W, int32_t H, int32_t first_sample, int32_t n_samples, int32_t spu) {
    const TilePixel q = wave_tiled_pixel(tiles ? tiles[blockIdx.x] : (int32_t)blockIdx.x, threadIdx.x, W);
    if (q.px >= W || q.py >= H) return;
    float4* texel = reinterpret_cast<float4*>(fb) + (size_t)q.py * W + q.px;
    float4* mtexel = MOMENTS ? reinterpret_cast<float4*>(moments) + (size_t)q.py * W + q.px : nullptr;
    float acc[4] = { 0.0f, 0.0f, 0.0f, 0.0f }, S[4] = { 0.0f, 0.0f, 0.0f, 0.0f };
    if (first_sample > 1) {
        unpack4(*texel, acc);
        if (MOMENTS) unpack4(*mtexel, S);
    }
    const float4* sb = reinterpret_cast<const float4*>(sbuf);
    for (int32_t k = 0; k < n_samples; ++k) {
        const int32_t chunk = k / spu, sl = k - chunk * spu;
        float L[4];
        unpack4(sb[pool_slot<size_t>((size_t)chunk, n_tiles, (size_t)blockIdx.x, (uint32_t)q.sub, spu, (size_t)sl, (uint32_t)q.lane)], L);
        fold_sample<MOMENTS>(acc, S, L, first_sample + k);
    }
    *texel = pack4(acc);
    if (MOMENTS) *mtexel = pack4(S);
}

template <bool MOMENTS>
__global__ void __launch_bounds__(256)
sky_kernel(const SceneParams P, float* __restrict__ fb, float* __restrict__ moments, const int32_t* __restrict__ tiles, int32_t first_sample, int32_t n_samples,
           const SeedTable seeds, uint32_t* __restrict__ status) {
    const int32_t W = P.u.resolution[0], H = P.u.resolution[1];
    const TilePixel q = wave_tiled_pixel(tiles[blockIdx.x], threadIdx.x, W);
    if (q.px >= W || q.py >= H) return;
    float4* texel = reinterpret_cast<float4*>(fb) + (size_t)q.py * W + q.px;
    float4* mtexel = MOMENTS ? reinterpret_cast<float4*>(moments) + (size_t)q.py * W + q.px : nullptr;
    float acc[4] = { 0.0f, 0.0f, 0.0f, 0.0f }, S[4] = { 0.0f, 0.0f, 0.0f, 0.0f };
    if (first_sample > 1) {
        unpack4(*texel, acc);
        if (MOMENTS) unpack4(*mtexel, S);
    }
    bool hit = false;
    for (int32_t k = 0; k < n_samples; ++k) {
        const int32_t smp = first_sample + k;
        uint32_t seed;
        if (seeds.table != nullptr && smp - 1 < seeds.cap) seed = seeds.table[seed_table_index<uint32_t>((uint32_t)(smp - 1), seeds.n_tiles, (uint32_t)q.tile, (uint32_t)q.sub, (uint32_t)q.lane)];
        else seed = path_seed((uint32_t)P.u.seed, W, q.px, q.py, smp);
        float L[4];
        if (!sky_sample(P, q.px, q.py, seed, L)) { hit = true; break; }
        fold_sample<MOMENTS>(acc, S, L, smp);
    }
    *texel = pack4(acc);
    if (MOMENTS) *mtexel = pack4(S);
    if (hit) atomicOr(status, kSkyHitStatus);
}

template <bool TF>
__global__ void __launch_bounds__(256)
features_kernel(const SceneParams P, const int32_t* __restrict__ tiles, int32_t spp, float* __restrict__ out, uint32_t* __restrict__ status) {
    const int32_t W = P.u.resolution[0], H = P.u.resolution[1];
    const TilePixel q = wave_tiled_pixel(tiles ? tiles[blockIdx.x] : (int32_t)blockIdx.x, threadIdx.x, W);
    if (q.px >= W || q.py >= H) return;
    float f[8];
    if (!feature_pixel<TF>(P, q.px, q.py, spp, f)) atomicOr(status, kFeatureLostStatus);
    float4* o = reinterpret_cast<float4*>(out) + 2u * ((size_t)q.py * W + q.px);
    o[0] = pack4(f);
    o[1] = pack4(f + 4);
}
void launch_features(const SceneParams& P, const int32_t* tiles, int32_t n_tiles, int32_t spp, float* out, uint32_t* status, hipStream_t stream) {
    if (n_tiles <= 0 || spp <= 0) return;
    if (P.u.use_tf) hipLaunchKernelGGL(features_kernel<true>, dim3((unsigned)n_tiles), dim3(256), 0, stream, P, tiles, spp, out, status);
    else hipLaunchKernelGGL(features_kernel<false>, dim3((unsigned)n_tiles), dim3(256), 0, stream, P, tiles, spp, out, status);
}

template <bool TF, bool SKIP, bool STATS>
__global__ void __launch_bounds__(256)
features_expected_kernel(const SceneParams P, const int32_t* __restrict__ tiles, int32_t rays, float* __restrict__ out, const ClearTable clear,
                         unsigned long long* __restrict__ stats) {
    const int32_t W = P.u.resolution[0], H = P.u.resolution[1];
    const TilePixel q = wave_tiled_pixel(tiles ? tiles[blockIdx.x] : (int32_t)blockIdx.x, threadIdx.x, W);
    const bool live = q.px < W && q.py < H;
    if (!STATS && !live) return;
    ExpectedWork work = { 0u, 0u, 0u, 0u, 0u };
    if (live) {
        float f[8];
        expected_pixel<TF, false, SKIP, STATS>(P, q.px, q.py, rays, f, nullptr, SKIP ? &clear : nullptr, STATS ? &work : nullptr);
        float4* o = reinterpret_cast<float4*>(out) + 2u * ((size_t)q.py * W + q.px);
        o[0] = pack4(f);
        o[1] = pack4(f + 4);
    }
    if (STATS) {
        uint32_t v[4] = { work.rays, work.steps, work.fetched, work.reads };
#pragma unroll
        for (int c = 0; c < 4; ++c)
            for (int o = 32; o > 0; o >>= 1) v[c] += (uint32_t)__shfl_xor((int)v[c], o);
        const uint32_t lane = threadIdx.x & 63u;
        if (lane < 4u) atomicAdd(stats + lane, (unsigned long long)(lane == 0u ? v[0] : (lane == 1u ? v[1] : (lane == 2u ? v[2] : v[3]))));
    }
}
void launch_features_expected(const SceneParams& P, const int32_t* tiles, int32_t n_tiles, int32_t rays, float* out, hipStream_t stream,
                              const ClearTable* clear, unsigned long long* stats) {
    if (n_tiles <= 0 || rays < 1 || rays > kExpectedMaxRays) return;
    const bool skip = clear && clear->d;
    const ClearTable C = skip ? *clear : ClearTable{ nullptr, { 0, 0, 0 } };
    const bool tf = P.u.use_tf != 0;
    const dim3 grid((unsigned)n_tiles), block(256);
#define VR_EXPECTED_LAUNCH(TF, SKIP, STATS) hipLaunchKernelGGL((features_expected_kernel<TF, SKIP, STATS>), grid, block, 0, stream, P, tiles, rays, out, C, stats)
    if (stats) {
        if (skip) { if (tf) VR_EXPECTED_LAUNCH(true, true, true); else VR_EXPECTED_LAUNCH(false, true, true); }
        else { if (tf) VR_EXPECTED_LAUNCH(true, false, true); else VR_EXPECTED_LAUNCH(false, false, true); }
    } else {
        if (skip) { if (tf) VR_EXPECTED_LAUNCH(true, true, false); else VR_EXPECTED_LAUNCH(false, true, false); }
        else { if (tf) VR_EXPECTED_LAUNCH(true, false, false); else VR_EXPECTED_LAUNCH(false, false, false); }
    }
#undef VR_EXPECTED_LAUNCH
}

static int32_t samples_per_unit(const PathtraceTuning& T, int32_t variant_default) { return T.samples_per_unit > 0 ? T.samples_per_unit : variant_default; }

PathtraceTuning default_tuning() {
    static std::once_flag once;
    static int32_t env_spu = 0, env_blocks = 0;
    std::call_once(once, [] {
        if (const char* e = getenv("VR_SPU")) env_spu = std::max(1, atoi(e));
        if (const char* e = getenv("VR_BLOCKS_PER_CU")) env_blocks = std::max(0, atoi(e));
    });
    PathtraceTuning T;
    T.samples_per_unit = env_spu;
    T.blocks_per_cu = env_blocks;
    return T;
}

size_t pathtrace_pool_floats(const PathtraceTuning& T, int32_t n_tiles, int32_t n_samples) {
    size_t padded = 0;
    for (int variant = 0; variant < kPtVariants; ++variant) {
        const int32_t spu = std::min(n_samples, samples_per_unit(T, pathtrace_unit_samples(variant)));
        padded = std::max(padded, (size_t)((n_samples + spu - 1) / spu) * (size_t)spu);
    }
    return padded * (size_t)n_tiles * 4u * 64u * 4u;
}

extern "C" {
#define VR_PT_DECL(N) \
    int vr_pt_occupancy_##N(int tf, int stats); \
    void vr_pt_launch_##N(int tf, int stats, unsigned grid, hipStream_t stream, const void* P, float* sbuf, float* cold_ws, const void* D, const void* S, uint32_t* status, unsigned long long* stats_buf, const void* seeds);
VR_PT_DECL(0) VR_PT_DECL(1) VR_PT_DECL(2) VR_PT_DECL(3) VR_PT_DECL(4) VR_PT_DECL(0_fast) VR_PT_DECL(1_fast) VR_PT_DECL(2_fast) VR_PT_DECL(3_fast) VR_PT_DECL(4_fast)
VR_PT_DECL(0w) VR_PT_DECL(1w) VR_PT_DECL(0w_fast) VR_PT_DECL(1w_fast)
#undef VR_PT_DECL
}
typedef int (*PtOccupancy)(int, int);
typedef void (*PtLaunch)(int, int, unsigned, hipStream_t, const void*, float*, float*, const void*, const void*, uint32_t*, unsigned long long*, const void*);
static const struct { PtOccupancy occupancy; PtLaunch launch; } kPtInstance[2][kPtInstances] = {
    { { vr_pt_occupancy_0, vr_pt_launch_0 }, { vr_pt_occupancy_0w, vr_pt_launch_0w }, { vr_pt_occupancy_1, vr_pt_launch_1 }, { vr_pt_occupancy_1w, vr_pt_launch_1w },
      { vr_pt_occupancy_2, vr_pt_launch_2 }, { vr_pt_occupancy_4, vr_pt_launch_4 }, { vr_pt_occupancy_3, vr_pt_launch_3 } },
    { { vr_pt_occupancy_0_fast, vr_pt_launch_0_fast }, { vr_pt_occupancy_0w_fast, vr_pt_launch_0w_fast }, { vr_pt_occupancy_1_fast, vr_pt_launch_1_fast }, { vr_pt_occupancy_1w_fast, vr_pt_launch_1w_fast },
      { vr_pt_occupancy_2_fast, vr_pt_launch_2_fast }, { vr_pt_occupancy_4_fast, vr_pt_launch_4_fast }, { vr_pt_occupancy_3_fast, vr_pt_launch_3_fast } } };

static void note_unexpected_reasons(int why) {
    if (why & (VR_VARIANT_ENV_DIVISION | VR_VARIANT_DENSITY_SCALE)) {
        static std::once_flag once;
        std::call_once(once, [&] {
            fprintf(stderr, "volren_amd: note: this scene is rendered by the run-time kernel variant (slower; results unchanged):%s%s\n",
                    (why & VR_VARIANT_ENV_DIVISION) ? " the environment's warp table has thresholds below 2^-76 (vr_get_int env_div_safe = 0);" : "",
                    (why & VR_VARIANT_DENSITY_SCALE) ? " the density scale lies outside [2^-16, 2^24];" : "");
        });
    }
}

static int resident_blocks(const PathtraceTuning& T, int mode, int instance, bool tf, bool stats) {
    int dev = 0, cus = 0;
    if (hipGetDevice(&dev) != hipSuccess) return 1024;
    static std::mutex mu;
    static std::map<uint32_t, std::pair<int, int>> cache;
    const uint32_t key = ((uint32_t)dev << 8) | ((uint32_t)mode << 5) | ((uint32_t)instance << 2) | (tf ? 2u : 0u) | (stats ? 1u : 0u);
    std::pair<int, int> v;
    {
        std::lock_guard<std::mutex> lock(mu);
        auto it = cache.find(key);
        if (it == cache.end()) {
            if (hipDeviceGetAttribute(&cus, hipDeviceAttributeMultiprocessorCount, dev) != hipSuccess || cus <= 0) cus = 256;
            it = cache.emplace(key, std::make_pair(cus, kPtInstance[mode][instance].occupancy(tf, stats))).first;
        }
        v = it->second;
    }
    const int per_cu = T.blocks_per_cu > 0 ? T.blocks_per_cu : v.second;
    return std::min(v.first * per_cu, kMaxWorkgroups * 4 / kWgWaves);
}

size_t pathtrace_workspace_floats() { return kColdMainFloats + (size_t)kMaxWorkgroups * 4u * (size_t)kColdSideWaveFloats; }

void launch_pathtrace(const PathtraceTuning& T, const SceneParams& P, float* fb, float* sample_pool, float* workspace, uint32_t* unit_counter, const int32_t* tiles, int32_t n_tiles,
                      int32_t first_sample, int32_t n_samples, uint32_t* status, hipStream_t stream, bool fast_math, hipEvent_t ev_kernel_begin, hipEvent_t ev_kernel_end,
                      float* moments, const uint32_t* seed_table, int32_t seed_samples, const int32_t* sky_tiles, int32_t n_sky_tiles) {
    if (n_samples <= 0 || (n_tiles <= 0 && n_sky_tiles <= 0)) return;
    SeedTable seeds;
    seeds.table = seed_samples > 0 ? seed_table : nullptr;
    seeds.cap = seed_samples;
    seeds.n_tiles = tile_count(P.u.resolution[0], P.u.resolution[1]);
    auto launch_sky = [&] {
        if (n_sky_tiles <= 0) return;
        const auto sky = moments ? sky_kernel<true> : sky_kernel<false>;
        hipLaunchKernelGGL(sky, dim3((unsigned)n_sky_tiles), dim3(256), 0, stream, P, fb, moments, sky_tiles, first_sample, n_samples, seeds, status);
    };
    if (n_tiles <= 0) {
        if (ev_kernel_begin) (void)hipEventRecord(ev_kernel_begin, stream);
        launch_sky();
        if (ev_kernel_end) (void)hipEventRecord(ev_kernel_end, stream);
        return;
    }
    SchedParams S;
    for (int i = 0; i < ST_COUNT; ++i) S.thr[i] = T.thr[i];
    LaunchDesc D;
    D.tiles = tiles; D.n_tiles = n_tiles; D.first_sample = first_sample; D.n_samples = n_samples;
    const bool tf = P.u.use_tf != 0, stats = T.stats != nullptr;
    const PathtraceKernel K = pathtrace_kernel_of(P, T.wide_addressing != 0, stats);
    note_unexpected_reasons(K.reason);
    D.spu = std::min(n_samples, samples_per_unit(T, K.samples_per_unit));
    const int32_t chunks = (n_samples + D.spu - 1) / D.spu;
    if ((uint64_t)chunks * (uint64_t)n_tiles * 4u * (uint64_t)(D.spu * 64) > 0xFFFFFFFFull)
        throw std::runtime_error("launch_pathtrace: " + std::to_string(n_tiles) + " tiles x " + std::to_string(n_samples) + " samples do not fit the 32-bit item index of one launch");
    D.n_units = (uint32_t)chunks * (uint32_t)n_tiles * 4u;
    D.chunks = (uint32_t)chunks;
    D.seg_len = (D.n_units + kQueueSegments - 1u) / kQueueSegments;
    D.unit_counter = unit_counter;
    S.max_iters = kMaxIdleIters;
    if (S.thr[ST_COLLIDE] <= 0) S.thr[ST_COLLIDE] = (P.u.use_tf || P.u.has_emission) ? 32 : 24;
    const int mode = fast_math ? 1 : 0;
    const int blocks = resident_blocks(T, mode, K.instance, tf, stats);
    const uint32_t groups_needed = (D.n_units + (uint32_t)kWgWaves - 1u) / (uint32_t)kWgWaves;
    const dim3 grid((unsigned)std::min<uint32_t>((uint32_t)blocks, groups_needed > 0 ? groups_needed : 1u)), block(256);
    if (K.item_integrator) {
        const uint64_t items = (uint64_t)D.n_units * (uint64_t)(D.spu * 64);
        const auto integrate = K.item_integrator == 2 ? item_kernel<2> : item_kernel<3>;
        hipLaunchKernelGGL(integrate, dim3((unsigned)((items + 255) / 256)), block, 0, stream, P, sample_pool, D);
        launch_sky();
    } else {
        (void)hipMemsetAsync(unit_counter, 0, kQueueSegments * sizeof(uint32_t), stream);
        if (ev_kernel_begin) (void)hipEventRecord(ev_kernel_begin, stream);
        kPtInstance[mode][K.instance].launch(tf, stats, grid.x, stream, &P, sample_pool, workspace, &D, &S, status, T.stats, &seeds);
        launch_sky();
        if (ev_kernel_end) (void)hipEventRecord(ev_kernel_end, stream);
    }
    const auto accumulate = moments ? accumulate_kernel<true> : accumulate_kernel<false>;
    hipLaunchKernelGGL(accumulate, dim3((unsigned)n_tiles), block, 0, stream, sample_pool, fb, moments, tiles, n_tiles, P.u.resolution[0], P.u.resolution[1],
                       first_sample, n_samples, D.spu);
}

}
```

volren_amd/csrc/vr_sky_tiles.h:

```cpp
#pragma once

#include <cmath>
#include <cstdint>
#include <vector>

#include "vr_scene.h"
#include "vr_tiles.h"

namespace vr {

constexpr double kSkyFrontMargin = 1e-3;
constexpr double kSkyPixelMargin = 1.0;

struct SkyProjection {
    bool valid = false;
    int n_axes = 0;
    double ax[30], ay[30], lo[30], hi[30];
};

inline SkyProjection sky_project_box(const SceneParams& P) {
    SkyProjection S;
    const Uniforms& u = P.u;
    const double W = (double)u.resolution[0], H = (double)u.resolution[1], cz = (double)P.cam_z;
    if (!(W >= 1.0) || !(H >= 1.0) || !std::isfinite(cz) || cz == 0.0) return S;
    double m[9], inv[9];
    for (int i = 0; i < 9; ++i) { m[i] = (double)u.cam_transform[i]; if (!std::isfinite(m[i])) return S; }
    const double c00 = m[4] * m[8] - m[7] * m[5], c01 = m[7] * m[2] - m[1] * m[8], c02 = m[1] * m[5] - m[4] * m[2];
    const double det = m[0] * c00 + m[3] * c01 + m[6] * c02;
    if (!std::isfinite(det) || det == 0.0) return S;
    inv[0] = c00 / det; inv[1] = c01 / det; inv[2] = c02 / det;
    inv[3] = (m[6] * m[5] - m[3] * m[8]) / det; inv[4] = (m[0] * m[8] - m[6] * m[2]) / det; inv[5] = (m[3] * m[2] - m[0] * m[5]) / det;
    inv[6] = (m[3] * m[7] - m[6] * m[4]) / det; inv[7] = (m[6] * m[1] - m[0] * m[7]) / det; inv[8] = (m[0] * m[4] - m[3] * m[1]) / det;
    double bb[2][3], cam[3];
    bool inside = true;
    for (int i = 0; i < 3; ++i) {
        bb[0][i] = (double)u.vol_bb_min[i]; bb[1][i] = (double)u.vol_bb_max[i]; cam[i] = (double)u.cam_pos[i];
        if (!std::isfinite(bb[0][i]) || !std::isfinite(bb[1][i]) || !std::isfinite(cam[i]) || bb[0][i] > bb[1][i]) return S;
        inside = inside && cam[i] >= bb[0][i] && cam[i] <= bb[1][i];
    }
    if (inside) return S;
    double X[8], Y[8];
    for (int k = 0; k < 8; ++k) {
        const double v[3] = { bb[k & 1][0] - cam[0], bb[(k >> 1) & 1][1] - cam[1], bb[(k >> 2) & 1][2] - cam[2] };
        const double lx = inv[0] * v[0] + inv[3] * v[1] + inv[6] * v[2], ly = inv[1] * v[0] + inv[4] * v[1] + inv[7] * v[2], lz = inv[2] * v[0] + inv[5] * v[1] + inv[8] * v[2];
        const double depth = lz / cz * std::fabs(cz);
        const double dist = std::sqrt(lx * lx + ly * ly + lz * lz);
        if (!std::isfinite(depth) || !std::isfinite(dist) || !(depth > 0.0) || !(depth >= kSkyFrontMargin * dist)) return S;
        X[k] = 0.5 * W + H * lx * cz / lz;
        Y[k] = 0.5 * H + H * ly * cz / lz;
        if (!std::isfinite(X[k]) || !std::isfinite(Y[k])) return S;
    }
    auto add_axis = [&](double ax, double ay) {
        if (ax == 0.0 && ay == 0.0) return;
        double lo = ax * X[0] + ay * Y[0], hi = lo;
        for (int k = 1; k < 8; ++k) { const double d = ax * X[k] + ay * Y[k]; lo = d < lo ? d : lo; hi = d > hi ? d : hi; }
        S.ax[S.n_axes] = ax; S.ay[S.n_axes] = ay; S.lo[S.n_axes] = lo; S.hi[S.n_axes] = hi;
        ++S.n_axes;
    };
    add_axis(1.0, 0.0);
    add_axis(0.0, 1.0);
    for (int a = 0; a < 8; ++a)
        for (int b = a + 1; b < 8; ++b) {
            const double ex = X[b] - X[a], ey = Y[b] - Y[a], len = std::sqrt(ex * ex + ey * ey);
            if (len > 0.0 && std::isfinite(len)) add_axis(-ey / len, ex / len);
        }
    S.valid = true;
    return S;
}

inline bool sky_tile_clear(const SkyProjection& S, int32_t W, int32_t H, int32_t tile) {
    if (!S.valid) return false;
    const int32_t nx = tiles_x(W), tx = tile % nx, ty = tile / nx;
    const double x0 = (double)(tx * 16) - kSkyPixelMargin, y0 = (double)(ty * 16) - kSkyPixelMargin;
    const double x1 = (double)(tx * 16 + 16 < W ? tx * 16 + 16 : W) + kSkyPixelMargin, y1 = (double)(ty * 16 + 16 < H ? ty * 16 + 16 : H) + kSkyPixelMargin;
    for (int i = 0; i < S.n_axes; ++i) {
        const double ax = S.ax[i], ay = S.ay[i];
        const double rlo = (ax >= 0.0 ? ax * x0 : ax * x1) + (ay >= 0.0 ? ay * y0 : ay * y1);
        const double rhi = (ax >= 0.0 ? ax * x1 : ax * x0) + (ay >= 0.0 ? ay * y1 : ay * y0);
        if (rhi < S.lo[i] || rlo > S.hi[i]) return true;
    }
    return false;
}

inline void sky_classify_tiles(const SceneParams& P, const int32_t* tiles, int32_t n, uint8_t* clear) {
    const SkyProjection S = sky_project_box(P);
    for (int32_t i = 0; i < n; ++i) clear[i] = sky_tile_clear(S, P.u.resolution[0], P.u.resolution[1], tiles[i]) ? 1 : 0;
}

inline void sky_split_tiles(const SceneParams& P, const std::vector<int32_t>& ids, int32_t n_tiles, std::vector<int32_t>& march, std::vector<int32_t>& sky) {
    march.clear(); sky.clear();
    const SkyProjection S = sky_project_box(P);
    const int32_t n = ids.empty() ? n_tiles : (int32_t)ids.size();
    for (int32_t i = 0; i < n; ++i) {
        const int32_t t = ids.empty() ? i : ids[(size_t)i];
        (sky_tile_clear(S, P.u.resolution[0], P.u.resolution[1], t) ? sky : march).push_back(t);
    }
}

}
```

volren_amd/csrc/vr_trace.h:

```cpp
#pragma once

#include <type_traits>

#include "vr_math.h"
#include "vr_scene.h"

#if defined(VR_HOST_TRACE) && !defined(__HIP_DEVICE_COMPILE__)
namespace vr {
enum TraceClass : int32_t { TR_MAJORANT = 0, TR_TAP = 1, TR_ENV_WARP = 2, TR_ENV_TEXEL = 3 };
void host_trace(int32_t cls, const void* table, size_t a, size_t b);
}
#define VR_TRACE(CLS, TABLE, A, B) ::vr::host_trace((CLS), (TABLE), (size_t)(A), (size_t)(B))
#else
#define VR_TRACE(CLS, TABLE, A, B) do { } while (0)
#endif

namespace vr {

enum LaneState : int32_t {
    ST_NEW = 0,
    ST_BEGIN = 1,
    ST_MARCH = 2,
    ST_COLLIDE = 3,
    ST_NEE = 4,
// ... 620 lines not shown
    return kInv4Pi * (1.0f - sqr(g)) / (denom * sqrt_(denom));
}
VR_HD v3 align(v3 N, v3 v) {
    const bool xa = abs_(N.x) > abs_(N.y);
    const float a = xa ? N.x : N.y;
    const v3 T = (xa ? v3{ -N.z, 0.0f, N.x } : v3{ 0.0f, N.z, -N.y }) / sqrt_(a * a + N.z * N.z);
    const v3 B = cross(N, T);
    return normalize(v3{ v.x * T.x + v.y * B.x + v.z * N.x,
                         v.x * T.y + v.y * B.y + v.z * N.y,
                         v.x * T.z + v.y * B.z + v.z * N.z });
}
VR_HD v3 sample_phase_hg(v3 dir, float g, float r0, float r1) {
    const float cos_t = abs_(g) < 1e-4f ? 1.0f - 2.0f * r0 :
        (1.0f + sqr(g) - sqr((1.0f - sqr(g)) / (1.0f - g + 2.0f * g * r0))) / (2.0f * g);
    const float sin_t = sqrt_(max_(0.0f, 1.0f - sqr(cos_t)));
    const float phi = 2.0f * kPi * r1;
    float sp, cp;
    sincos_(phi, sp, cp);
    return align(dir, v3{ sin_t * cp, sin_t * sp, cos_t });
}
VR_HD float power_heuristic(float a, float b) { return sqr(a) / (sqr(a) + sqr(b)); }

VR_HD v3 rcp3_exact(v3 v) {
#if defined(__HIP_DEVICE_COMPILE__) && !VR_FAST_DEVICE
    v3 r = v3{ rcp_newton(v.x), rcp_newton(v.y), rcp_newton(v.z) };
    if (!((int)rcp_in_fast_range(v.x) & (int)rcp_in_fast_range(v.y) & (int)rcp_in_fast_range(v.z))) r = v3{ 1.0f / v.x, 1.0f / v.y, 1.0f / v.z };
    return r;
#else
    return v3{ 1.0f / v.x, 1.0f / v.y, 1.0f / v.z };
#endif
}

VR_HD bool intersect_box(v3 pos, v3 dir, const float* bmin, const float* bmax, float& tnear, float& tfar) {
    const v3 inv = rcp3_exact(dir);
    const v3 lo = (v3{ bmin[0], bmin[1], bmin[2] } - pos) * inv;
    const v3 hi = (v3{ bmax[0], bmax[1], bmax[2] } - pos) * inv;
    const v3 tmin = v3{ min_(lo.x, hi.x), min_(lo.y, hi.y), min_(lo.z, hi.z) };
    const v3 tmax = v3{ max_(lo.x, hi.x), max_(lo.y, hi.y), max_(lo.z, hi.z) };
    tnear = max_(0.0f, max_(tmin.x, max_(tmin.y, tmin.z)));
    tfar = min_(tmax.x, min_(tmax.y, tmax.z));
    return tnear <= tfar;
}

template <bool CLEAN = false>
VR_HD float step_dda(v3 p, v3 ri, int32_t mip) {
    const float dim = u2f((uint32_t)(130 + mip) << 23);
    const float idim = u2f((uint32_t)(124 - mip) << 23);
    const float ox = ri.x >= 0.0f ? dim + 0.5f : -0.5f;
    const float oy = ri.y >= 0.0f ? dim + 0.5f : -0.5f;
    const float oz = ri.z >= 0.0f ? dim + 0.5f : -0.5f;
    const float tx = (floor_(p.x * idim) * dim + ox - p.x) * ri.x;
    const float ty = (floor_(p.y * idim) * dim + oy - p.y) * ri.y;
    const float tz = (floor_(p.z * idim) * dim + oz - p.z) * ri.z;
    if (CLEAN) return __builtin_fminf(tx, __builtin_fminf(ty, tz));
    return min_(tx, min_(ty, tz));
}


VR_HD void hot_init(Hot& h) {
    h.seed = 0u; h.item = 0u;
    h.ipos = h.idir = h.ri = h.ethr = h.eL = h.shle = h.wpos = h.wdir = v3{ 0, 0, 0 };
    h.t = h.far = h.tau = h.majorant = h.Tr = 0.0f;
    h.mipq = 0;
    h.shadow = 0;
    h.state = ST_NEW;
    h.first = 0;
    h.maj_idx = -2; h.maj_raw = 0u;
}

VR_HD void write_sample(const WorkUnit& wu, uint32_t item, v3 L, uint32_t n_paths) {
    float* o = wu.out + 4u * (size_t)item;
#if defined(__HIP_DEVICE_COMPILE__)
    typedef float vr_f4 __attribute__((ext_vector_type(4)));
    __builtin_nontemporal_store(vr_f4{ L.x, L.y, L.z, n_paths > 0u ? 1.0f : 0.0f }, reinterpret_cast<vr_f4*>(o));
#else
    o[0] = L.x; o[1] = L.y; o[2] = L.z; o[3] = n_paths > 0u ? 1.0f : 0.0f;
#endif
}

VR_HD void accumulate_sample(float acc[4], const float L[4], int32_t current_sample) {
    const float a = 1.0f / (float)current_sample;
    acc[0] = mix_(acc[0], sanitize(L[0]), a);
    acc[1] = mix_(acc[1], sanitize(L[1]), a);
    acc[2] = mix_(acc[2], sanitize(L[2]), a);
    acc[3] = mix_(acc[3], sanitize(L[3]), a);
}

template <class K>
VR_HD bool begin_segment(Hot& h, const SceneParams& P, v3 pos, v3 d, int32_t shadow) {
    h.wpos = pos; h.wdir = d;
    h.shadow = shadow;
    h.Tr = 1.0f;
    h.mipq = 12;
    float tnear, tfar;
    if (!intersect_box(pos, d, P.u.vol_bb_min, P.u.vol_bb_max, tnear, tfar)) {
        h.state = segment_end_state(shadow);
        return false;
    }
    h.ipos = mat4_point(P.u.vol_density_inv_transform, pos);
    h.idir = mat4_dir(P.u.vol_density_inv_transform, d);
    h.far = tfar;
    if (K::global == 2 ? P.u.integrator != 0 : K::global == 1) {
        h.ri = v3{ 0, 0, 0 };
        h.tau = 0.0f;
        h.far = -tfar;
        h.t = tnear + neg_log_1m(rng(h.seed)) * P.u.vol_inv_majorant;
        if (h.t < tfar) { h.majorant = P.u.vol_majorant; h.state = ST_COLLIDE; }
        else h.state = segment_end_state(shadow);
        return true;
    }
    h.ri = rcp3_exact(h.idir);
    h.t = tnear + 1e-6f;
    h.tau = neg_log_1m(rng(h.seed));
    h.state = ST_MARCH;
    {
        const float ax = abs_(h.idir.x), ay = abs_(h.idir.y), az = abs_(h.idir.z), amax = __builtin_fmaxf(ax, __builtin_fmaxf(ay, az));
        const bool clean = (int)(abs_(h.ipos.x) < kCleanBound) & (int)(abs_(h.ipos.y) < kCleanBound) & (int)(abs_(h.ipos.z) < kCleanBound) &
                           (int)(ax * tfar < kCleanBound) & (int)(ay * tfar < kCleanBound) & (int)(az * tfar < kCleanBound) &
                           (int)(amax < kCleanBound) & (int)(amax >= 1.0f / kCleanBound);
        h.far = clean ? tfar : -tfar;
    }
    return true;
}

template <class K, class Cold, bool LAZY_EM = false>
VR_HD void do_new(Hot& h, Cold& c, const SceneParams& P, const WorkUnit& wu, uint32_t item, bool have_seed = false, uint32_t table_seed = 0u) {
    const int32_t W = P.u.resolution[0], H = P.u.resolution[1];
    const int32_t px = wu.px0 + (int32_t)(item & 7u), py = wu.py0 + (int32_t)((item >> 3) & 7u);
    const int32_t smp = wu.first_sample + (int32_t)(item >> 6);
    if (px >= W || py >= H) return;
    if (have_seed) h.seed = table_seed;
    else h.seed = path_seed((uint32_t)P.u.seed, W, px, py, smp);
    const float jx = rng(h.seed), jy = rng(h.seed);
    const float fx = (((float)px + jx) - (float)W * 0.5f) / (float)H;
    const float fy = (((float)py + jy) - (float)H * 0.5f) / (float)H;
    const v3 dir = normalize(mat3_mul(P.u.cam_transform, normalize(v3{ fx, fy, P.cam_z })));
    const v3 pos = v3{ P.u.cam_pos[0], P.u.cam_pos[1], P.u.cam_pos[2] };
    const bool hit = begin_segment<K>(h, P, pos, dir, 0);
    const bool lazy = LAZY_EM || !hit || !(K::emission == 2 ? P.u.has_emission != 0 : K::emission == 1);
    if (!lazy) {
        st3(c, C_POS, pos); st3(c, C_DIR, dir);
        st3(c, C_L, v3{ 0, 0, 0 }); st3(c, C_THR, v3{ 1, 1, 1 });
        stu(c, C_NPATHS, 0u); c.st(C_FP, 0.0f); stu(c, C_ITEM, wu.base + item);
    }
    h.first = lazy ? 1 : 0;
    h.ipos = v3{ lazy ? dir.x : h.ipos.x, lazy ? dir.y : h.ipos.y, lazy ? dir.z : h.ipos.z };
    h.Tr = lazy ? u2f(wu.base + item) : h.Tr;
}
VR_HD void first_resume(Hot& h, const SceneParams& P) {
    h.ipos = mat4_point(P.u.vol_density_inv_transform, v3{ P.u.cam_pos[0], P.u.cam_pos[1], P.u.cam_pos[2] });
    h.Tr = 1.0f;
}

VR_HD bool sky_sample(const SceneParams& P, int32_t px, int32_t py, uint32_t seed, float out[4]) {
    const int32_t W = P.u.resolution[0], H = P.u.resolution[1];
    const float jx = rng(seed), jy = rng(seed);
    const float fx = (((float)px + jx) - (float)W * 0.5f) / (float)H;
    const float fy = (((float)py + jy) - (float)H * 0.5f) / (float)H;
    const v3 dir = normalize(mat3_mul(P.u.cam_transform, normalize(v3{ fx, fy, P.cam_z })));
    const v3 pos = v3{ P.u.cam_pos[0], P.u.cam_pos[1], P.u.cam_pos[2] };
    float tnear, tfar;
    if (intersect_box(pos, dir, P.u.vol_bb_min, P.u.vol_bb_max, tnear, tfar)) return false;
    v3 L = v3{ 0.0f, 0.0f, 0.0f };
    if (P.u.show_environment > 0) L = L + (v3{ 1.0f, 1.0f, 1.0f } * 1.0f) * lookup_environment(P, dir);
    out[0] = L.x; out[1] = L.y; out[2] = L.z; out[3] = 0.0f;
    return true;
}

struct MarchIO { float dt1, dt2, t1; uint32_t maj1, maj2; int32_t i1, i2; bool go1, go2; };
VR_HD void march_idle(MarchIO& io) { io.i1 = io.i2 = 0; io.dt1 = io.dt2 = io.t1 = 0.0f; io.go1 = io.go2 = false; }
template <int DENSE = 2, int MAJB = 2, bool CLEAN = false>
VR_HD void march_prep(const Hot& h, const SceneParams& P, MarchIO& io) {
    const float far = seg_far(h);
    io.go1 = h.t < far;
    const v3 c1 = axpy(h.ipos, h.t, h.idir);
    const int32_t m1 = round_mip_q(h.mipq);
    io.i1 = majorant_index<DENSE, MAJB, CLEAN>(P.density, c1, m1);
    io.dt1 = step_dda<CLEAN>(c1, h.ri, m1);
    io.t1 = h.t + io.dt1;
    const int32_t q2 = h.mipq < 12 ? h.mipq + 1 : 12;
    const int32_t m2 = round_mip_q(q2);
    io.go2 = io.t1 < far;
    const v3 c2 = axpy(h.ipos, io.t1, h.idir);
    io.i2 = majorant_index<DENSE, MAJB, CLEAN>(P.density, c2, m2);
    io.dt2 = step_dda<CLEAN>(c2, h.ri, m2);
}
template <bool TF, bool A32 = false>
VR_HD void march_load(const SceneParams& P, MarchIO& io) {
    io.maj1 = majorant_fetch<TF, A32>(P.density, io.i1);
    io.maj2 = majorant_fetch<TF, A32>(P.density, io.i2);
}
template <bool TF, bool A32 = false>
VR_HD void march_load_reuse(const SceneParams& P, MarchIO& io, const Hot& h) {
    const bool same = io.i1 == h.maj_idx;
    const uint32_t m1 = majorant_fetch<TF, A32>(P.density, same ? 0 : io.i1);
    io.maj1 = same ? h.maj_raw : m1;
    io.maj2 = majorant_fetch<TF, A32>(P.density, io.i2);
}
template <bool TF, bool REUSE = false, bool CLEAN = false>
VR_HD void march_finish(Hot& h, const SceneParams& P, const MarchIO& io) {
    if (!io.go1) { h.state = segment_end_state(h.shadow); return; }
    float t = io.t1, maj = majorant_value<TF>(P, io.maj1);
    float tau = h.tau - maj * io.dt1;
    int32_t q = h.mipq < 12 ? h.mipq + 1 : 12;
    if (REUSE) { h.maj_idx = io.i1; h.maj_raw = io.maj1; }
    if (tau > 0.0f) {
        if (!io.go2) { h.t = t; h.tau = tau; h.mipq = q; h.state = segment_end_state(h.shadow); return; }
        maj = majorant_value<TF>(P, io.maj2);
        if (REUSE) { h.maj_idx = io.i2; h.maj_raw = io.maj2; }
        t = io.t1 + io.dt2;
        tau = tau - maj * io.dt2;
        q = q < 12 ? q + 1 : 12;
        if (tau > 0.0f) { h.t = t; h.tau = tau; h.mipq = q; return; }
    }
    t += (CLEAN && !TF) ? div_core(tau, maj) : tau / maj;
    h.t = t; h.tau = tau; h.mipq = q;
    if (t >= seg_far(h)) { h.state = segment_end_state(h.shadow); return; }
    h.majorant = maj;
    h.state = ST_COLLIDE;
}
template <bool TF, int DENSE = 2, int MAJB = 2>
VR_HD void do_march(Hot& h, const SceneParams& P) {
    if (!(h.t < seg_far(h))) { h.state = segment_end_state(h.shadow); return; }
    const v3 curr = axpy(h.ipos, h.t, h.idir);
    const int32_t m = round_mip_q(h.mipq);
    const float majorant = majorant_at<TF, DENSE, MAJB>(P, curr, m);
    const float dt = step_dda(curr, h.ri, m);
    h.t += dt;
    h.tau -= majorant * dt;
    h.mipq = h.mipq < 12 ? h.mipq + 1 : 12;
    if (h.tau > 0.0f) return;
    h.t += h.tau / majorant;
    if (h.t >= seg_far(h)) { h.state = segment_end_state(h.shadow); return; }
    h.majorant = majorant;
    h.state = ST_COLLIDE;
}

template <class K> struct CollideIO {
    TapAddr a; TapData d;
    TriIO tri;
    TapAddr ea; TapData ed;
};
template <class K, bool CLEAN = false>
VR_HD void collide_prep(Hot& h, const SceneParams& P, const SceneParams& PE, CollideIO<K>& io) {
    const v3 ip = axpy(h.ipos, h.t, h.idir);
    if (K::tf) {
        trilinear_prep<K::dense, !CLEAN>(P.density, ip, io.tri);
    } else {
        int32_t tx, ty, tz;
        tricubic_tap<!CLEAN>(ip, h.seed, tx, ty, tz);
        io.a = tap_addr<K::dense>(P.density, tx, ty, tz);
    }
    io.ea.cell = io.ea.off = 0u; io.ea.in = false;
    if (!h.shadow) {
        if (K::emission == 2 ? P.u.has_emission != 0 : K::emission == 1) {
            const v3 ie = mat4_point(PE.emission_from_density, ip);
            int32_t ex, ey, ez;
            tricubic_tap(ie, h.seed, ex, ey, ez);
            io.ea = tap_addr<K::edense>(PE.emission, ex, ey, ez);
        } else {
            rng_skip9(h.seed);
        }
    }
}
template <class K>
VR_HD void collide_idle(CollideIO<K>& io) {
    io.a.cell = io.a.off = 0u; io.a.in = false;
    io.ea.cell = io.ea.off = 0u; io.ea.in = false;
    if (K::tf) trilinear_idle(io.tri);
}
template <class K, bool CLEAN = false>
VR_HD void collide_prep(Hot& h, const SceneParams& P, CollideIO<K>& io) { collide_prep<K, CLEAN>(h, P, P, io); }
template <class K>
VR_HD void collide_load(const SceneParams& P, const SceneParams& PE, CollideIO<K>& io) {
    if (K::tf) trilinear_load<K::dense, K::pair_d, K::a32>(P.density, io.tri);
    else io.d = tap_load<K::dense, K::pair_d, K::a32>(P.density, io.a);
    if (K::emission == 2 ? P.u.has_emission != 0 : K::emission == 1) io.ed = tap_load<K::edense, K::pair_e, K::a32>(PE.emission, io.ea);
}
template <class K>
VR_HD void collide_load(const SceneParams& P, CollideIO<K>& io) { collide_load<K>(P, P, io); }
#ifndef VR_SHADOW_BLOCKED_SHORTCUT
#define VR_SHADOW_BLOCKED_SHORTCUT (!VR_FAST_DEVICE)
#endif
template <class K>
VR_HD void collide_tail_pin(CollideIO<K>& io, uint32_t& s1, uint32_t& s2, float& r1, float& tau2, float& vol_majorant) {
#if defined(__HIP_DEVICE_COMPILE__)
    if (K::tf) {
        asm volatile("" : "+v"(io.tri.d[0].raw), "+v"(io.tri.d[1].raw), "+v"(io.tri.d[2].raw), "+v"(io.tri.d[3].raw), "+v"(io.tri.d[4].raw), "+v"(io.tri.d[5].raw),
                          "+v"(io.tri.d[6].raw), "+v"(io.tri.d[7].raw), "+v"(s1), "+v"(s2), "+v"(r1), "+v"(tau2), "+s"(vol_majorant));
    } else {
        asm volatile("" : "+v"(io.d.raw), "+v"(s1), "+v"(s2), "+v"(r1), "+v"(tau2), "+s"(vol_majorant));
    }
#endif
}
template <class K, class Cold, bool CACHED = false, bool EARLY = false>
VR_HD void collide_finish(Hot& h, Cold& c, const SceneParams& P, const SceneParams& PE, const CollideIO<K>& io_in, const float* tf_lut) {
    static_assert(!EARLY || K::global == 0, "the early tail is the DDA trackers'");
    constexpr bool USE_TF = K::tf;
    const Uniforms& u = P.u;
    const bool global = K::global == 2 ? u.integrator != 0 : K::global == 1;
    std::conditional_t<EARLY, CollideIO<K>, const CollideIO<K>&> io = io_in;
    uint32_t s1 = h.seed, s2 = 0u;
    float r1 = 0.0f, tau2 = 0.0f, vm = u.vol_majorant;
    bool premises = false;
    if constexpr (EARLY) {
        r1 = rng(s1);
        s2 = s1;
        tau2 = neg_log_1m(rng(s2));
        collide_tail_pin<K>(io, s1, s2, r1, tau2, vm);
#if VR_SHADOW_BLOCKED_SHORTCUT
        premises = (h.majorant > 0.0f) & (h.majorant <= vm) & (abs_(h.Tr) < inf_());
#endif
    }
    float d;
    float rgba[4] = { 0, 0, 0, 0 };
// ... 486 lines not shown
```

volren_amd/renderer.py:

```python
import ctypes as C

import numpy as np

from . import _lib

_INT_FIELDS = ("sample", "sppx", "seed", "bounces", "show_environment", "tonemapping", "integrator", "grid_frame_counter",
               "sample_pool_mb", "gpu_encoder", "fast_math", "tf_float_atlas", "launch_target_ms", "order_tiles", "coalesce_trace", "majorant_layout",
               "variance", "denoise_iterations", "denoise_moments", "denoise_resolve", "denoise_layers", "denoise_filter", "wide_addressing", "seed_table_mb", "seed_table_max_samples",
               "expected_skip", "expected_stats", "sky_tiles")
_READ_ONLY_INT_FIELDS = ("n_grid_frames", "last_launches", "last_sky_tiles", "pending_samples", "majorant_blocked", "env_div_safe", "env_compact", "kernel_variant", "kernel_variant_reason",
                         "kernel_wide", "adaptive_rounds", "seed_table_samples", "seed_table_fills")
_FLOAT_FIELDS = {"tonemap_exposure": 1, "tonemap_gamma": 1, "albedo": 3, "phase": 1, "density_scale": 1,
                 "emission_scale": 1, "vol_clip_min": 3, "vol_clip_max": 3, "env_strength": 1, "env_transform": 9,
                 "tf_window_left": 1, "tf_window_width": 1, "cam_pos": 3, "cam_dir": 3, "cam_up": 3, "cam_fov": 1,
                 "volume_transform": 16, "denoise_sigma": 5, "denoise_alpha": 1, "denoise_reject": 1, "denoise_ridge": 1}


def _f32(a):
    return np.ascontiguousarray(a, dtype=np.float32)


class Renderer:

    def __init__(self, width, height, device=0, _borrowed=None):
        object.__setattr__(self, "_h", None)
        L = _lib.load()
        object.__setattr__(self, "_owned", _borrowed is None)
        if _borrowed is None:
            h = C.c_void_p()
            _lib.check(L.vr_create(C.byref(h), int(device), int(width), int(height)))
        else:
            h = C.c_void_p(_borrowed)
        object.__setattr__(self, "_h", h)
        object.__setattr__(self, "_L", L)
        object.__setattr__(self, "width", int(width))
        object.__setattr__(self, "height", int(height))

    def close(self):
        if self._h is not None:
            if self._owned:
                self._L.vr_destroy(self._h)
            object.__setattr__(self, "_h", None)

    def __del__(self):
        try:
            self.close()
        except Exception:
            pass

    def get_int(self, name):
        v = C.c_int()
        _lib.check(self._L.vr_get_int(self._h, name.encode(), C.byref(v)))
        return v.value

    def __getattr__(self, name):
        if name in _INT_FIELDS or name in _READ_ONLY_INT_FIELDS:
            v = self.get_int(name)
            return bool(v) if name in ("show_environment", "tonemapping") else v
        if name in _FLOAT_FIELDS:
            n = _FLOAT_FIELDS[name]
            buf = (C.c_float * n)()
            _lib.check(self._L.vr_get_float(self._h, name.encode(), buf, n))
            return buf[0] if n == 1 else np.array(buf[:], np.float32)
        raise AttributeError(name)

    def __setattr__(self, name, value):
        if name in _INT_FIELDS:
            _lib.check(self._L.vr_set_int(self._h, name.encode(), int(value)))
        elif name in _FLOAT_FIELDS or name == "env_rot":
            v = _f32(np.atleast_1d(value)).reshape(-1)
            _lib.check(self._L.vr_set_float(self._h, name.encode(), v.ctypes.data_as(C.POINTER(C.c_float)), v.size))
        else:
            object.__setattr__(self, name, value)

    def has_fast_math(self):
        return True

    def load_volume(self, path):
        _lib.check(self._L.vr_load_volume(self._h, str(path).encode()))

    def set_volume_path(self, path):
        _lib.check(self._L.vr_set_volume_path(self._h, str(path).encode()))

    def volume_aabb(self, name="density"):
        out = (C.c_float * 6)()
        _lib.check(self._L.vr_volume_aabb(self._h, name.encode(), out))
        return np.array(out[:3], np.float32), np.array(out[3:], np.float32)

    def volume_minorant_majorant(self, name="density"):
        out = (C.c_float * 2)()
        _lib.check(self._L.vr_volume_minorant_majorant(self._h, name.encode(), out))
        return float(out[0]), float(out[1])

    def load_envmap(self, path):
        _lib.check(self._L.vr_load_envmap(self._h, str(path).encode()))

    def load_transferfunc(self, path):
        _lib.check(self._L.vr_load_transferfunc(self._h, str(path).encode()))

    def set_volume_dense(self, voxels_zyx, transform=None, name="density", unit_cube=True, commit=True):
        v = _f32(voxels_zyx)
        nz, ny, nx = v.shape
        t = _f32(transform).reshape(16) if transform is not None else None
        _lib.check(self._L.vr_set_volume_dense(self._h, name.encode(), v.ctypes.data, nx, ny, nz,
                                               t.ctypes.data if t is not None else None, 1 if unit_cube else 0))
        if commit:
            self.commit()

    def volume_add_grid_frame(self, voxels_zyx, name="density", transform=None):
        v = _f32(voxels_zyx)
        nz, ny, nx = v.shape
        t = _f32(transform).reshape(16) if transform is not None else None
        _lib.check(self._L.vr_volume_add_grid_frame_dense(self._h, name.encode(), v.ctypes.data, nx, ny, nz, t.ctypes.data if t is not None else None))

    def volume_update_grid_frame(self, frame, voxels_zyx, name="density", transform=None):
        v = _f32(voxels_zyx)
        nz, ny, nx = v.shape
        t = _f32(transform).reshape(16) if transform is not None else None
        _lib.check(self._L.vr_volume_update_grid_frame_dense(self._h, int(frame), name.encode(), v.ctypes.data, nx, ny, nz, t.ctypes.data if t is not None else None))

    def volume_n_grid_frames(self):
        n = C.c_int()
        _lib.check(self._L.vr_volume_n_grid_frames(self._h, C.byref(n)))
        return n.value

    def set_volume_dense_f16(self, voxels_zyx, transform=None, name="density", unit_cube=True, commit=True):
        v = np.ascontiguousarray(voxels_zyx, dtype=np.float16)
        nz, ny, nx = v.shape
        t = _f32(transform).reshape(16) if transform is not None else None
        _lib.check(self._L.vr_set_volume_dense_f16(self._h, name.encode(), v.ctypes.data, nx, ny, nz,
                                                   t.ctypes.data if t is not None else None, 1 if unit_cube else 0))
        if commit:
            self.commit()

    def set_volume_brick(self, transform, n_bricks, min_maj, indirection, rng, atlas_dim, atlas, mips=(), name="density",
                         unit_cube=True, commit=True):
        t = _f32(transform).reshape(16)
        nb = np.asarray(n_bricks, np.uint32)
        mm = _f32(min_maj)
        ind = np.ascontiguousarray(indirection, np.uint32)
        rg = np.ascontiguousarray(rng, np.uint32)
        ad = np.asarray(atlas_dim, np.uint32)
        at = np.ascontiguousarray(atlas, np.uint8)
        mip_arrays = [np.ascontiguousarray(a, np.uint32) for _, a in mips]
        mip_ptrs = (C.c_void_p * max(1, len(mips)))(*[a.ctypes.data for a in mip_arrays])
        mip_dims = np.asarray([d for d, _ in mips], np.uint32).reshape(-1, 3) if mips else np.zeros((1, 3), np.uint32)
        _lib.check(self._L.vr_set_volume_brick(self._h, name.encode(), t.ctypes.data, nb.ctypes.data, mm.ctypes.data,
                                               ind.ctypes.data, rg.ctypes.data, ad.ctypes.data, at.ctypes.data,
                                               len(mips), C.cast(mip_ptrs, C.c_void_p), mip_dims.ctypes.data, 1 if unit_cube else 0))
        if commit:
            self.commit()

    def set_envmap(self, rgb_top_first):
        a = _f32(rgb_top_first)
        _lib.check(self._L.vr_set_envmap(self._h, a.ctypes.data, a.shape[1], a.shape[0]))

    def set_transferfunc(self, lut):
        if lut is None:
            _lib.check(self._L.vr_set_transferfunc(self._h, None, 0))
            return
        a = _f32(lut)
        _lib.check(self._L.vr_set_transferfunc(self._h, a.ctypes.data, a.shape[0]))

# ... 443 lines not shown
```

Baseline: 5857 Msamples/s.

## Render tiles whose rays cross only empty volume cells with the sky kernel

At commit time a host-side hierarchy of non-empty density cells is built. When tiles are split, that hierarchy is projected to screen tiles to find tiles whose camera rays cross the bounding box but never reach a voxel with density. Those tiles are sent to the cheap sky kernel with the box test skipped, instead of through the path tracer. This adds a conservative CPU traversal at each split-key change and extra cache-key inputs. Correctness relies on the projection margins being conservative, and it only applies to the non-emissive integrators without a transfer function.

```diff
diff --git a/volren_amd/csrc/capi.cpp b/volren_amd/csrc/capi.cpp
--- a/volren_amd/csrc/capi.cpp
+++ b/volren_amd/csrc/capi.cpp
@@ -119,6 +119,8 @@
     { "order_tiles", VR_INT(order_tiles), 0, 2, "order_tiles: 0 (never), 1 (tile subsets), 2 (always)" },
     { "sky_tiles", VR_INT(sky_tiles), 0, 1, "sky_tiles: 0 (every tile through the path tracer) or 1 (tiles whose camera rays cannot hit the volume's box are rendered apart)" },
     { "last_sky_tiles", VR_READ_ONLY(R.last_sky_tiles) },
+    { "see_through_tiles", VR_INT(see_through_tiles), 0, 1, "see_through_tiles: 0 or 1 (where the clear tiles are rendered apart, so are the tiles whose camera rays cross the box without reaching a voxel with density)" },
+    { "last_see_through_tiles", VR_READ_ONLY(R.last_see_through_tiles) },
     { "grid_frame_counter", VR_GET(R.volume ? (int)R.volume->grid_frame_counter : 0), set_grid_frame, VR_ANY },
     { "n_grid_frames", VR_READ_ONLY(R.volume ? (int)R.volume->n_grid_frames() : 0) },
     { "last_launches", VR_READ_ONLY(R.last_launches) },
diff --git a/volren_amd/csrc/renderer.cpp b/volren_amd/csrc/renderer.cpp
--- a/volren_amd/csrc/renderer.cpp
+++ b/volren_amd/csrc/renderer.cpp
@@ -79,11 +79,16 @@
     emission_grids.clear();
     majorant_emission = 0.f;
     maj_key_ = MajKey{};
+    ++commit_version_;
     std::cout << "Preparing brick grids for HIP..." << std::endl;
     std::vector<size_t> with_emission;
     for (const auto& frame : volume->grids) {
         Volume::GridPtr density_grid = frame.at("density");
         density_grids.push_back(grid_to_device(density_grid));
+        if (auto bg = std::dynamic_pointer_cast<BrickGrid>(density_grid))
+            density_grids.back().live_cells = std::make_shared<const SkyLiveCells>(sky_live_cells(bg->range.data.data(), (int32_t)bg->range.stride.x, (int32_t)bg->range.stride.y, (int32_t)bg->range.stride.z));
+        else if (auto dg = std::dynamic_pointer_cast<DenseGridF16>(density_grid))
+            density_grids.back().live_cells = std::make_shared<const SkyLiveCells>(sky_live_cells(dg->range.data.data(), (int32_t)dg->range.stride.x, (int32_t)dg->range.stride.y, (int32_t)dg->range.stride.z));
         Volume::GridPtr emission_grid;
         for (const char* name : { "flame", "flames", "temperature" }) {
             auto it = frame.find(name);
@@ -464,26 +469,44 @@
     return key ? key : 1;
 }
 
-RendererHIP::SplitTiles RendererHIP::split_tiles(const SceneParams& P, const std::vector<int32_t>& ids, int n_tiles, bool ordered) {
+void RendererHIP::split_three(const LaunchInputs& in, const std::vector<int32_t>& ids, int n_tiles, std::vector<int32_t>& march, std::vector<int32_t>& clear, std::vector<int32_t>& see) const {
+    static const SkyLiveCells none;
+    const std::shared_ptr<const SkyLiveCells>& held = density_grids.at(in.frame).live_cells;
+    sky_split_tiles3(in.P, in.see_through_tiles != 0 && held ? *held : none, ids, n_tiles, march, clear, see);
+}
+
+RendererHIP::SplitTiles RendererHIP::split_tiles(const LaunchInputs& in, const std::vector<int32_t>& ids, int n_tiles, bool ordered) {
+    const SceneParams& P = in.P;
     const int tag = ordered ? 2 : 1;
     uint64_t key = fnv1a(&tag, sizeof tag, tile_order_key(P, ids, n_tiles));
+    {
+        const Uniforms& u = P.u;
+        const uint64_t frame = in.frame, version = commit_version_;
+        auto mix = [&key](const void* p, size_t nbytes) { key = fnv1a(p, nbytes, key); };
+        mix(&frame, sizeof frame); mix(&version, sizeof version); mix(&in.see_through_tiles, sizeof in.see_through_tiles);
+        mix(u.vol_density_transform, sizeof u.vol_density_transform); mix(&u.vol_density_scale, sizeof u.vol_density_scale);
+        mix(&u.integrator, sizeof u.integrator); mix(&u.has_emission, sizeof u.has_emission); mix(&u.use_tf, sizeof u.use_tf);
+    }
     key = key ? key : 1;
     if (split_key_ != key) {
-        std::vector<int32_t> march, sky;
-        sky_split_tiles(P, ids, n_tiles, march, sky);
-        if (!sky.empty()) {
+        std::vector<int32_t> march, clear, see;
+        split_three(in, ids, n_tiles, march, clear, see);
+        if (!clear.empty() || !see.empty()) {
             if (ordered && !march.empty()) march = costliest_first(P, march, (int)march.size());
-            march.insert(march.end(), sky.begin(), sky.end());
+            march.insert(march.end(), clear.begin(), clear.end());
+            march.insert(march.end(), see.begin(), see.end());
             ensure_buffer(split_dev_, march.size() * sizeof(int32_t));
             split_dev_->upload(march.data(), march.size() * sizeof(int32_t), stream);
         }
-        split_n_sky_ = (int)sky.size();
+        split_n_sky_ = (int)clear.size();
+        split_n_see_ = (int)see.size();
         split_key_ = key;
     }
     SplitTiles s;
-    if (split_n_sky_ > 0) {
+    if (split_n_sky_ + split_n_see_ > 0) {
         s.n_sky = split_n_sky_;
-        s.n_march = n_tiles - split_n_sky_;
+        s.n_see = split_n_see_;
+        s.n_march = n_tiles - split_n_sky_ - split_n_see_;
         s.march = split_dev_->as<int32_t>();
         s.sky = s.march + s.n_march;
     }
@@ -502,7 +525,7 @@
 
 bool RendererHIP::LaunchInputs::same_launch_as(const LaunchInputs& o) const {
     return memcmp(&P, &o.P, sizeof P) == 0 && frame == o.frame && maj == o.maj && tuning == o.tuning && order_tiles == o.order_tiles && launch_target_ms == o.launch_target_ms &&
-           fast_math == o.fast_math && variance == o.variance && sky_tiles == o.sky_tiles && sample_pool_bytes == o.sample_pool_bytes && stream == o.stream;
+           fast_math == o.fast_math && variance == o.variance && sky_tiles == o.sky_tiles && see_through_tiles == o.see_through_tiles && sample_pool_bytes == o.sample_pool_bytes && stream == o.stream;
 }
 
 void RendererHIP::capture(LaunchInputs& in) {
@@ -548,6 +571,7 @@
     in.maj.blocked = in.P.density.maj_blocked;
     in.tuning = tuning;
     in.order_tiles = order_tiles; in.launch_target_ms = launch_target_ms; in.fast_math = fast_math ? 1 : 0; in.variance = variance != 0 ? 1 : 0; in.sky_tiles = sky_tiles != 0 ? 1 : 0;
+    in.see_through_tiles = see_through_tiles != 0 ? 1 : 0;
     in.sample_pool_bytes = sample_pool_bytes;
     in.stream = stream;
     in.env = environment; in.tf = transferfunc;
@@ -569,11 +593,11 @@
     if (n <= 0) return;
     const int n_tiles = tile_set_size();
     const bool ordered = in.order_tiles >= 2 || (in.order_tiles == 1 && tiles_dev_);
-    const SplitTiles split = in.splits_sky() ? split_tiles(in.P, tiles_dev_ ? tiles_host_ : std::vector<int32_t>(), n_tiles, ordered) : SplitTiles{};
-    if (split.n_sky > 0) {
-        const int per_launch = prepare_submit(in, first, n, split.n_march, split.n_sky);
+    const SplitTiles split = in.splits_sky() ? split_tiles(in, tiles_dev_ ? tiles_host_ : std::vector<int32_t>(), n_tiles, ordered) : SplitTiles{};
+    if (split.n_sky + split.n_see > 0) {
+        const int per_launch = prepare_submit(in, first, n, split.n_march, split.n_sky + split.n_see);
         open_timing_window(in.stream);
-        submit(in, first, n, split.march, split.n_march, per_launch, split.sky, split.n_sky);
+        submit(in, first, n, split.march, split.n_march, per_launch, split.sky, split.n_sky, split.n_see);
         close_timing_window(in.stream);
         return;
     }
@@ -623,13 +647,14 @@
     return per_launch;
 }
 
-void RendererHIP::submit(const LaunchInputs& in, int first, int n, const int32_t* tiles, int n_tiles, int per_launch, const int32_t* sky, int n_sky) {
+void RendererHIP::submit(const LaunchInputs& in, int first, int n, const int32_t* tiles, int n_tiles, int per_launch, const int32_t* sky, int n_sky, int n_see) {
     const SceneParams& P = in.P;
     last_sky_tiles = n_sky;
+    last_see_through_tiles = n_see;
     hipStream_t stream = in.stream;
     const PathtraceKernel kernel = in.kernel();
     const bool pt_kernel = kernel.item_integrator == 0;
-    const double px_samples = (double)(n_tiles + n_sky) * 256.0;
+    const double px_samples = (double)(n_tiles + n_sky + n_see) * 256.0;
     const uint64_t key = [&] {
         uint64_t h = kFnv1aStart;
         auto mix = [&h](const void* p, size_t nbytes) { h = fnv1a(p, nbytes, h); };
@@ -670,7 +695,7 @@
         int seed_samples = 0;
         const uint32_t* seed_table = kernel.reads_seed_table ? seed_table_for(P, first + done, m, stream, &seed_samples) : nullptr;
         launch_pathtrace(in.tuning, P, color->as<float>(), n_tiles > 0 ? pool_->as<float>() : nullptr, n_tiles > 0 ? workspace_->as<float>() : nullptr, status_->as<uint32_t>() + 1, tiles, n_tiles, first + 1 + done, m,
-                         status_->as<uint32_t>(), stream, in.fast_math != 0, eb, ee, moments, seed_table, seed_samples, sky, n_sky);
+                         status_->as<uint32_t>(), stream, in.fast_math != 0, eb, ee, moments, seed_table, seed_samples, sky, n_sky, n_see);
         VR_HIP(hipGetLastError());
         done += m;
         if (pt_kernel) { rate_pending_samples_ = px_samples * (double)m; rate_pending_key_ = key; }
@@ -1420,23 +1445,26 @@
     auto launch_groups = [&](const std::vector<int32_t>& ids, const auto& to) {
         const auto groups = adaptive_groups(ids, tile_n_);
         std::vector<int32_t> packed;
-        std::vector<int> n_sky;
+        std::vector<int> n_sky, n_see;
         for (const auto& g : groups) {
-            std::vector<int32_t> march = g.second, sky;
-            if (split) sky_split_tiles(in.P, g.second, (int)g.second.size(), march, sky);
+            std::vector<int32_t> march = g.second, sky, see;
+            if (split) split_three(in, g.second, (int)g.second.size(), march, sky, see);
             if (ordered && !march.empty()) march = costliest_first(in.P, march, (int)march.size());
             packed.insert(packed.end(), march.begin(), march.end());
             packed.insert(packed.end(), sky.begin(), sky.end());
+            packed.insert(packed.end(), see.begin(), see.end());
             n_sky.push_back((int)sky.size());
+            n_see.push_back((int)see.size());
         }
         if (packed.empty()) return;
         sized_.adaptive_lists->upload(packed.data(), packed.size() * sizeof(int32_t), in.stream);
         size_t off = 0, k = 0;
         for (const auto& g : groups) {
             const int32_t n = g.first, next = to(n);
-            const int n_clear = n_sky[k++], n_tiles = (int)g.second.size() - n_clear;
+            const int n_clear = n_sky[k], n_through = n_see[k], n_tiles = (int)g.second.size() - n_clear - n_through;
+            ++k;
             const int32_t* list = sized_.adaptive_lists->as<int32_t>() + off;
-            submit(in, n, next - n, list, n_tiles, prepare_submit(in, n, next - n, n_tiles, n_clear), n_clear > 0 ? list + n_tiles : nullptr, n_clear);
+            submit(in, n, next - n, list, n_tiles, prepare_submit(in, n, next - n, n_tiles, n_clear + n_through), n_clear + n_through > 0 ? list + n_tiles : nullptr, n_clear, n_through);
             for (int32_t t : g.second) tile_n_[(size_t)t] = next;
             off += g.second.size();
         }
diff --git a/volren_amd/csrc/renderer.h b/volren_amd/csrc/renderer.h
--- a/volren_amd/csrc/renderer.h
+++ b/volren_amd/csrc/renderer.h
@@ -14,6 +14,8 @@
 #include "vr_scene.h"
 
 namespace vr {
+
+struct SkyLiveCells;
 
 struct Camera {
     vec3 pos{ 1.f, 0.f, 1.f };
@@ -44,6 +46,7 @@
     int32_t mshift[3] = { 3, 3, 3 };
     size_t n_active = 0;
     bool maj_blocked = false;
+    std::shared_ptr<const SkyLiveCells> live_cells;
     mat4 transform;
 };
 
@@ -116,6 +119,8 @@
     PathtraceTuning tuning = default_tuning();
     int sky_tiles = 1;
     int last_sky_tiles = 0;
+    int see_through_tiles = 1;
+    int last_see_through_tiles = 0;
     int last_launches = 0;
     int adaptive_rounds = 0;
     int launch_target_ms = 2000;
@@ -198,7 +203,7 @@
         MajKey maj;
         size_t frame = 0;
         PathtraceTuning tuning;
-        int order_tiles = 0, launch_target_ms = 0, fast_math = 0, variance = 0, sky_tiles = 0;
+        int order_tiles = 0, launch_target_ms = 0, fast_math = 0, variance = 0, sky_tiles = 0, see_through_tiles = 0;
         size_t sample_pool_bytes = 0;
         hipStream_t stream = nullptr;
         std::shared_ptr<Environment> env;
@@ -210,7 +215,7 @@
     };
     void capture(LaunchInputs& in);
     int prepare_submit(const LaunchInputs& in, int first, int n, int n_tiles, int n_sky = 0);
-    void submit(const LaunchInputs& in, int first, int n, const int32_t* tiles, int n_tiles, int per_launch, const int32_t* sky = nullptr, int n_sky = 0);
+    void submit(const LaunchInputs& in, int first, int n, const int32_t* tiles, int n_tiles, int per_launch, const int32_t* sky = nullptr, int n_sky = 0, int n_see = 0);
     void submit_tile_set(const LaunchInputs& in, int first, int n);
     void open_timing_window(hipStream_t s), close_timing_window(hipStream_t s);
     int tile_set_size() const;
@@ -226,11 +231,13 @@
     std::vector<int32_t> costliest_first(const SceneParams& P, const std::vector<int32_t>& ids, int n_tiles) const;
     const int32_t* tile_order(const SceneParams& P, const std::vector<int32_t>& ids, int n_tiles);
     uint64_t tile_order_key(const SceneParams& P, const std::vector<int32_t>& ids, int n_tiles) const;
-    struct SplitTiles { const int32_t* march = nullptr; int n_march = 0; const int32_t* sky = nullptr; int n_sky = 0; };
-    SplitTiles split_tiles(const SceneParams& P, const std::vector<int32_t>& ids, int n_tiles, bool ordered);
+    struct SplitTiles { const int32_t* march = nullptr; int n_march = 0; const int32_t* sky = nullptr; int n_sky = 0, n_see = 0; };
+    SplitTiles split_tiles(const LaunchInputs& in, const std::vector<int32_t>& ids, int n_tiles, bool ordered);
+    void split_three(const LaunchInputs& in, const std::vector<int32_t>& ids, int n_tiles, std::vector<int32_t>& march, std::vector<int32_t>& clear, std::vector<int32_t>& see) const;
     DeviceBufferPtr split_dev_;
     uint64_t split_key_ = 0;
-    int split_n_sky_ = 0;
+    int split_n_sky_ = 0, split_n_see_ = 0;
+    uint64_t commit_version_ = 0;
     std::vector<int32_t> tile_n_;
     int tile_n_sample_ = -1;
     DeviceBufferPtr status_;
diff --git a/volren_amd/csrc/vr_device.h b/volren_amd/csrc/vr_device.h
--- a/volren_amd/csrc/vr_device.h
+++ b/volren_amd/csrc/vr_device.h
@@ -30,7 +30,7 @@
                       hipEvent_t ev_kernel_begin = nullptr, hipEvent_t ev_kernel_end = nullptr,
                       float* moments = nullptr,
                       const uint32_t* seed_table = nullptr, int32_t seed_samples = 0,
-                      const int32_t* sky_tiles = nullptr, int32_t n_sky_tiles = 0);
+                      const int32_t* sky_tiles = nullptr, int32_t n_sky_tiles = 0, int32_t n_see_tiles = 0);
 constexpr uint32_t kSkyHitStatus = 8u;
 constexpr uint32_t kFeatureLostStatus = 4u;
 void launch_features(const SceneParams& P, const int32_t* tiles, int32_t n_tiles, int32_t spp, float* out, uint32_t* status, hipStream_t stream);
diff --git a/volren_amd/csrc/vr_launch.hip b/volren_amd/csrc/vr_launch.hip
--- a/volren_amd/csrc/vr_launch.hip
+++ b/volren_amd/csrc/vr_launch.hip
@@ -67,9 +67,10 @@
 
 template <bool MOMENTS>
 __global__ void __launch_bounds__(256)
-sky_kernel(const SceneParams P, float* __restrict__ fb, float* __restrict__ moments, const int32_t* __restrict__ tiles, int32_t first_sample, int32_t n_samples,
-           const SeedTable seeds, uint32_t* __restrict__ status) {
+sky_kernel(const SceneParams P, float* __restrict__ fb, float* __restrict__ moments, const int32_t* __restrict__ tiles, int32_t n_clear, int32_t first_sample,
+           int32_t n_samples, const SeedTable seeds, uint32_t* __restrict__ status) {
     const int32_t W = P.u.resolution[0], H = P.u.resolution[1];
+    const bool box_test = (int32_t)blockIdx.x < n_clear;
     const TilePixel q = wave_tiled_pixel(tiles[blockIdx.x], threadIdx.x, W);
     if (q.px >= W || q.py >= H) return;
     float4* texel = reinterpret_cast<float4*>(fb) + (size_t)q.py * W + q.px;
@@ -86,7 +87,7 @@
         if (seeds.table != nullptr && smp - 1 < seeds.cap) seed = seeds.table[seed_table_index<uint32_t>((uint32_t)(smp - 1), seeds.n_tiles, (uint32_t)q.tile, (uint32_t)q.sub, (uint32_t)q.lane)];
         else seed = path_seed((uint32_t)P.u.seed, W, q.px, q.py, smp);
         float L[4];
-        if (!sky_sample(P, q.px, q.py, seed, L)) { hit = true; break; }
+        if (!sky_sample(P, q.px, q.py, seed, L, box_test)) { hit = true; break; }
         fold_sample<MOMENTS>(acc, S, L, smp);
     }
     *texel = pack4(acc);
@@ -230,16 +231,16 @@
 
 void launch_pathtrace(const PathtraceTuning& T, const SceneParams& P, float* fb, float* sample_pool, float* workspace, uint32_t* unit_counter, const int32_t* tiles, int32_t n_tiles,
                       int32_t first_sample, int32_t n_samples, uint32_t* status, hipStream_t stream, bool fast_math, hipEvent_t ev_kernel_begin, hipEvent_t ev_kernel_end,
-                      float* moments, const uint32_t* seed_table, int32_t seed_samples, const int32_t* sky_tiles, int32_t n_sky_tiles) {
-    if (n_samples <= 0 || (n_tiles <= 0 && n_sky_tiles <= 0)) return;
+                      float* moments, const uint32_t* seed_table, int32_t seed_samples, const int32_t* sky_tiles, int32_t n_sky_tiles, int32_t n_see_tiles) {
+    if (n_samples <= 0 || (n_tiles <= 0 && n_sky_tiles + n_see_tiles <= 0)) return;
     SeedTable seeds;
     seeds.table = seed_samples > 0 ? seed_table : nullptr;
     seeds.cap = seed_samples;
     seeds.n_tiles = tile_count(P.u.resolution[0], P.u.resolution[1]);
     auto launch_sky = [&] {
-        if (n_sky_tiles <= 0) return;
+        if (n_sky_tiles + n_see_tiles <= 0) return;
         const auto sky = moments ? sky_kernel<true> : sky_kernel<false>;
-        hipLaunchKernelGGL(sky, dim3((unsigned)n_sky_tiles), dim3(256), 0, stream, P, fb, moments, sky_tiles, first_sample, n_samples, seeds, status);
+        hipLaunchKernelGGL(sky, dim3((unsigned)(n_sky_tiles + n_see_tiles)), dim3(256), 0, stream, P, fb, moments, sky_tiles, n_sky_tiles, first_sample, n_samples, seeds, status);
     };
     if (n_tiles <= 0) {
         if (ev_kernel_begin) (void)hipEventRecord(ev_kernel_begin, stream);
diff --git a/volren_amd/csrc/vr_sky_tiles.h b/volren_amd/csrc/vr_sky_tiles.h
--- a/volren_amd/csrc/vr_sky_tiles.h
+++ b/volren_amd/csrc/vr_sky_tiles.h
@@ -11,6 +11,43 @@
 
 constexpr double kSkyFrontMargin = 1e-3;
 constexpr double kSkyPixelMargin = 1.0;
+
+struct SkyCamera {
+    bool valid = false;
+    double W = 0.0, H = 0.0, cz = 0.0, inv[9], cam[3];
+};
+
+inline SkyCamera sky_camera(const SceneParams& P) {
+    SkyCamera C;
+    const Uniforms& u = P.u;
+    const double W = (double)u.resolution[0], H = (double)u.resolution[1], cz = (double)P.cam_z;
+    if (!(W >= 1.0) || !(H >= 1.0) || !std::isfinite(cz) || cz == 0.0) return C;
+    double m[9];
+    double* inv = C.inv;
+    for (int i = 0; i < 9; ++i) { m[i] = (double)u.cam_transform[i]; if (!std::isfinite(m[i])) return C; }
+    const double c00 = m[4] * m[8] - m[7] * m[5], c01 = m[7] * m[2] - m[1] * m[8], c02 = m[1] * m[5] - m[4] * m[2];
+    const double det = m[0] * c00 + m[3] * c01 + m[6] * c02;
+    if (!std::isfinite(det) || det == 0.0) return C;
+    inv[0] = c00 / det; inv[1] = c01 / det; inv[2] = c02 / det;
+    inv[3] = (m[6] * m[5] - m[3] * m[8]) / det; inv[4] = (m[0] * m[8] - m[6] * m[2]) / det; inv[5] = (m[3] * m[2] - m[0] * m[5]) / det;
+    inv[6] = (m[3] * m[7] - m[6] * m[4]) / det; inv[7] = (m[6] * m[1] - m[0] * m[7]) / det; inv[8] = (m[0] * m[4] - m[3] * m[1]) / det;
+    for (int i = 0; i < 3; ++i) { C.cam[i] = (double)u.cam_pos[i]; if (!std::isfinite(C.cam[i])) return C; }
+    C.W = W; C.H = H; C.cz = cz;
+    C.valid = true;
+    return C;
+}
+
+inline bool sky_project_point(const SkyCamera& C, const double c[3], double& X, double& Y) {
+    const double* inv = C.inv;
+    const double v[3] = { c[0] - C.cam[0], c[1] - C.cam[1], c[2] - C.cam[2] };
+    const double lx = inv[0] * v[0] + inv[3] * v[1] + inv[6] * v[2], ly = inv[1] * v[0] + inv[4] * v[1] + inv[7] * v[2], lz = inv[2] * v[0] + inv[5] * v[1] + inv[8] * v[2];
+    const double depth = lz / C.cz * std::fabs(C.cz);
+    const double dist = std::sqrt(lx * lx + ly * ly + lz * lz);
+    if (!std::isfinite(depth) || !std::isfinite(dist) || !(depth > 0.0) || !(depth >= kSkyFrontMargin * dist)) return false;
+    X = 0.5 * C.W + C.H * lx * C.cz / lz;
+    Y = 0.5 * C.H + C.H * ly * C.cz / lz;
+    return std::isfinite(X) && std::isfinite(Y);
+}
 
 struct SkyProjection {
     bool valid = false;
@@ -18,37 +55,26 @@
     double ax[30], ay[30], lo[30], hi[30];
 };
 
+inline bool sky_camera_in_box(const SkyCamera& C, const Uniforms& u, double bb[2][3]) {
+    bool inside = true;
+    for (int i = 0; i < 3; ++i) {
+        bb[0][i] = (double)u.vol_bb_min[i]; bb[1][i] = (double)u.vol_bb_max[i];
+        if (!std::isfinite(bb[0][i]) || !std::isfinite(bb[1][i]) || bb[0][i] > bb[1][i]) return true;
+        inside = inside && C.cam[i] >= bb[0][i] && C.cam[i] <= bb[1][i];
+    }
+    return inside;
+}
+
 inline SkyProjection sky_project_box(const SceneParams& P) {
     SkyProjection S;
-    const Uniforms& u = P.u;
-    const double W = (double)u.resolution[0], H = (double)u.resolution[1], cz = (double)P.cam_z;
-    if (!(W >= 1.0) || !(H >= 1.0) || !std::isfinite(cz) || cz == 0.0) return S;
-    double m[9], inv[9];
-    for (int i = 0; i < 9; ++i) { m[i] = (double)u.cam_transform[i]; if (!std::isfinite(m[i])) return S; }
-    const double c00 = m[4] * m[8] - m[7] * m[5], c01 = m[7] * m[2] - m[1] * m[8], c02 = m[1] * m[5] - m[4] * m[2];
-    const double det = m[0] * c00 + m[3] * c01 + m[6] * c02;
-    if (!std::isfinite(det) || det == 0.0) return S;
-    inv[0] = c00 / det; inv[1] = c01 / det; inv[2] = c02 / det;
-    inv[3] = (m[6] * m[5] - m[3] * m[8]) / det; inv[4] = (m[0] * m[8] - m[6] * m[2]) / det; inv[5] = (m[3] * m[2] - m[0] * m[5]) / det;
-    inv[6] = (m[3] * m[7] - m[6] * m[4]) / det; inv[7] = (m[6] * m[1] - m[0] * m[7]) / det; inv[8] = (m[0] * m[4] - m[3] * m[1]) / det;
-    double bb[2][3], cam[3];
-    bool inside = true;
-    for (int i = 0; i < 3; ++i) {
-        bb[0][i] = (double)u.vol_bb_min[i]; bb[1][i] = (double)u.vol_bb_max[i]; cam[i] = (double)u.cam_pos[i];
-        if (!std::isfinite(bb[0][i]) || !std::isfinite(bb[1][i]) || !std::isfinite(cam[i]) || bb[0][i] > bb[1][i]) return S;
-        inside = inside && cam[i] >= bb[0][i] && cam[i] <= bb[1][i];
-    }
-    if (inside) return S;
+    const SkyCamera C = sky_camera(P);
+    if (!C.valid) return S;
+    double bb[2][3];
+    if (sky_camera_in_box(C, P.u, bb)) return S;
     double X[8], Y[8];
     for (int k = 0; k < 8; ++k) {
-        const double v[3] = { bb[k & 1][0] - cam[0], bb[(k >> 1) & 1][1] - cam[1], bb[(k >> 2) & 1][2] - cam[2] };
-        const double lx = inv[0] * v[0] + inv[3] * v[1] + inv[6] * v[2], ly = inv[1] * v[0] + inv[4] * v[1] + inv[7] * v[2], lz = inv[2] * v[0] + inv[5] * v[1] + inv[8] * v[2];
-        const double depth = lz / cz * std::fabs(cz);
-        const double dist = std::sqrt(lx * lx + ly * ly + lz * lz);
-        if (!std::isfinite(depth) || !std::isfinite(dist) || !(depth > 0.0) || !(depth >= kSkyFrontMargin * dist)) return S;
-        X[k] = 0.5 * W + H * lx * cz / lz;
-        Y[k] = 0.5 * H + H * ly * cz / lz;
-        if (!std::isfinite(X[k]) || !std::isfinite(Y[k])) return S;
+        const double c[3] = { bb[k & 1][0], bb[(k >> 1) & 1][1], bb[(k >> 2) & 1][2] };
+        if (!sky_project_point(C, c, X[k], Y[k])) return S;
     }
     auto add_axis = [&](double ax, double ay) {
         if (ax == 0.0 && ay == 0.0) return;
@@ -68,11 +94,12 @@
     return S;
 }
 
-inline bool sky_tile_clear(const SkyProjection& S, int32_t W, int32_t H, int32_t tile) {
+inline bool sky_tile_apart(const SkyProjection& S, int32_t W, int32_t H, int32_t tile, double margin) {
     if (!S.valid) return false;
     const int32_t nx = tiles_x(W), tx = tile % nx, ty = tile / nx;
-    const double x0 = (double)(tx * 16) - kSkyPixelMargin, y0 = (double)(ty * 16) - kSkyPixelMargin;
-    const double x1 = (double)(tx * 16 + 16 < W ? tx * 16 + 16 : W) + kSkyPixelMargin, y1 = (double)(ty * 16 + 16 < H ? ty * 16 + 16 : H) + kSkyPixelMargin;
+    const double x0 = (double)(tx * 16) - margin, y0 = (double)(ty * 16) - margin;
+    const double x1 = (double)(tx * 16 + 16 < W ? tx * 16 + 16 : W) + margin, y1 = (double)(ty * 16 + 16 < H ? ty * 16 + 16 : H) + margin;
+    if (x0 > x1 || y0 > y1) return true;
     for (int i = 0; i < S.n_axes; ++i) {
         const double ax = S.ax[i], ay = S.ay[i];
         const double rlo = (ax >= 0.0 ? ax * x0 : ax * x1) + (ay >= 0.0 ? ay * y0 : ay * y1);
@@ -81,6 +108,8 @@
     }
     return false;
 }
+inline bool sky_tile_clear(const SkyProjection& S, int32_t W, int32_t H, int32_t tile) { return sky_tile_apart(S, W, H, tile, kSkyPixelMargin); }
+inline bool sky_tile_crossed(const SkyProjection& S, int32_t W, int32_t H, int32_t tile) { return S.valid && !sky_tile_apart(S, W, H, tile, -kSkyPixelMargin); }
 
 inline void sky_classify_tiles(const SceneParams& P, const int32_t* tiles, int32_t n, uint8_t* clear) {
     const SkyProjection S = sky_project_box(P);
@@ -97,4 +126,146 @@
     }
 }
 
-}
+constexpr double kSkyTapReach = 2.5;
+constexpr double kSkyCellGrow = kSkyTapReach + 1.0;
+
+inline bool sky_half_dead(uint32_t h) { h &= 0xFFFFu; return (h & 0x7FFFu) == 0u || ((h & 0x8000u) != 0u && (h & 0x7C00u) != 0x7C00u); }
+inline bool sky_half_nan(uint32_t h) { return (h & 0x7C00u) == 0x7C00u && (h & 0x03FFu) != 0u; }
+
+struct SkyLiveCells {
+    bool held = false;
+    bool nan = false;
+    std::vector<std::vector<uint8_t>> live;
+    std::vector<int32_t> n;
+};
+
+inline SkyLiveCells sky_live_cells(const uint32_t* range, int32_t nx, int32_t ny, int32_t nz) {
+    SkyLiveCells L;
+    if (!range || nx <= 0 || ny <= 0 || nz <= 0) return L;
+    L.held = true;
+    const size_t n0 = (size_t)nx * (size_t)ny * (size_t)nz;
+    L.live.emplace_back(n0);
+    L.n = { nx, ny, nz };
+    for (size_t i = 0; i < n0; ++i) {
+        const uint32_t w = range[i];
+        L.nan = L.nan || sky_half_nan(w) || sky_half_nan(w >> 16);
+        L.live[0][i] = (sky_half_dead(w) && sky_half_dead(w >> 16)) ? 0 : 1;
+    }
+    for (size_t m = 0; L.n[3 * m] > 1 || L.n[3 * m + 1] > 1 || L.n[3 * m + 2] > 1; ++m) {
+        const int32_t sx = L.n[3 * m], sy = L.n[3 * m + 1], sz = L.n[3 * m + 2];
+        const int32_t dx = (sx + 1) / 2, dy = (sy + 1) / 2, dz = (sz + 1) / 2;
+        std::vector<uint8_t> dst((size_t)dx * (size_t)dy * (size_t)dz, 0);
+        const std::vector<uint8_t>& src = L.live[m];
+        for (int32_t z = 0; z < sz; ++z)
+            for (int32_t y = 0; y < sy; ++y)
+                for (int32_t x = 0; x < sx; ++x)
+                    if (src[((size_t)z * sy + y) * sx + x]) dst[((size_t)(z >> 1) * dy + (y >> 1)) * dx + (x >> 1)] = 1;
+        L.live.push_back(std::move(dst));
+        L.n.push_back(dx); L.n.push_back(dy); L.n.push_back(dz);
+    }
+    return L;
+}
+
+inline bool sky_see_through_scene(const Uniforms& u) {
+    return (u.integrator == 0 || u.integrator == 1) && u.has_emission == 0 && u.use_tf == 0 && std::isfinite(u.vol_density_scale) && u.vol_density_scale >= 0.0f;
+}
+
+struct SkyTouched {
+    bool valid = false;
+    int32_t nx = 0, ny = 0;
+    std::vector<uint8_t> tile;
+    int64_t cells_visited = 0;
+};
+
+inline SkyTouched sky_touched_tiles(const SceneParams& P, const SkyLiveCells& L) {
+    SkyTouched T;
+    const Uniforms& u = P.u;
+    if (!L.held || L.nan || !sky_see_through_scene(u)) return T;
+    const SkyCamera C = sky_camera(P);
+    if (!C.valid) return T;
+    double bb[2][3];
+    if (sky_camera_in_box(C, u, bb)) return T;
+    double xf[16];
+    for (int i = 0; i < 16; ++i) { xf[i] = (double)u.vol_density_transform[i]; if (!std::isfinite(xf[i])) return T; }
+    T.nx = tiles_x(u.resolution[0]); T.ny = tiles_y(u.resolution[1]);
+    T.tile.assign((size_t)T.nx * (size_t)T.ny, 0);
+    struct Cell { int32_t m, x, y, z; };
+    std::vector<Cell> stack;
+    const int32_t top = (int32_t)L.live.size() - 1;
+    stack.push_back(Cell{ top, 0, 0, 0 });
+    while (!stack.empty()) {
+        const Cell c = stack.back();
+        stack.pop_back();
+        const int32_t sx = L.n[3 * (size_t)c.m], sy = L.n[3 * (size_t)c.m + 1];
+        ++T.cells_visited;
+        if (!L.live[(size_t)c.m][((size_t)c.z * sy + c.y) * sx + c.x]) continue;
+        const double s = (double)(8 << c.m);
+        const double lo[3] = { c.x * s - kSkyCellGrow, c.y * s - kSkyCellGrow, c.z * s - kSkyCellGrow };
+        const double hi[3] = { (c.x + 1) * s + kSkyCellGrow, (c.y + 1) * s + kSkyCellGrow, (c.z + 1) * s + kSkyCellGrow };
+        bool front = true;
+        double X0 = 0.0, X1 = 0.0, Y0 = 0.0, Y1 = 0.0;
+        for (int k = 0; k < 8 && front; ++k) {
+            const double ip[3] = { (k & 1) ? hi[0] : lo[0], (k & 2) ? hi[1] : lo[1], (k & 4) ? hi[2] : lo[2] };
+            double w[3], X, Y;
+            for (int r = 0; r < 3; ++r) w[r] = xf[r] * ip[0] + xf[4 + r] * ip[1] + xf[8 + r] * ip[2] + xf[12 + r];
+            front = sky_project_point(C, w, X, Y);
+            if (!front) break;
+            if (k == 0) { X0 = X1 = X; Y0 = Y1 = Y; }
+            else { X0 = X < X0 ? X : X0; X1 = X > X1 ? X : X1; Y0 = Y < Y0 ? Y : Y0; Y1 = Y > Y1 ? Y : Y1; }
+        }
+        bool descend = !front;
+        if (!front && c.m == 0) return SkyTouched{};
+        if (front) {
+            const double fx0 = std::ceil((X0 - kSkyPixelMargin) / 16.0) - 1.0, fx1 = std::floor((X1 + kSkyPixelMargin) / 16.0);
+            const double fy0 = std::ceil((Y0 - kSkyPixelMargin) / 16.0) - 1.0, fy1 = std::floor((Y1 + kSkyPixelMargin) / 16.0);
+            if (fx1 < 0.0 || fy1 < 0.0 || fx0 > (double)(T.nx - 1) || fy0 > (double)(T.ny - 1)) continue;
+            const int32_t tx0 = fx0 < 0.0 ? 0 : (int32_t)fx0, tx1 = fx1 > (double)(T.nx - 1) ? T.nx - 1 : (int32_t)fx1;
+            const int32_t ty0 = fy0 < 0.0 ? 0 : (int32_t)fy0, ty1 = fy1 > (double)(T.ny - 1) ? T.ny - 1 : (int32_t)fy1;
+            bool all_marked = true;
+            for (int32_t ty = ty0; ty <= ty1 && all_marked; ++ty)
+                for (int32_t tx = tx0; tx <= tx1; ++tx)
+                    if (!T.tile[(size_t)ty * T.nx + tx]) { all_marked = false; break; }
+            if (all_marked) continue;
+            if (c.m == 0 || (tx0 == tx1 && ty0 == ty1)) {
+                for (int32_t ty = ty0; ty <= ty1; ++ty)
+                    for (int32_t tx = tx0; tx <= tx1; ++tx) T.tile[(size_t)ty * T.nx + tx] = 1;
+                continue;
+            }
+            descend = true;
+        }
+        if (descend) {
+            const int32_t cx = L.n[3 * (size_t)(c.m - 1)], cy = L.n[3 * (size_t)(c.m - 1) + 1], cz = L.n[3 * (size_t)(c.m - 1) + 2];
+            for (int k = 0; k < 8; ++k) {
+                const int32_t x = 2 * c.x + (k & 1), y = 2 * c.y + ((k >> 1) & 1), z = 2 * c.z + (k >> 2);
+                if (x < cx && y < cy && z < cz) stack.push_back(Cell{ c.m - 1, x, y, z });
+            }
+        }
+    }
+    T.valid = true;
+    return T;
+}
+
+enum : uint8_t { kSkyMarch = 0, kSkyClear = 1, kSkySeeThrough = 2 };
+inline void sky_classify_tiles3(const SceneParams& P, const SkyLiveCells& L, const int32_t* tiles, int32_t n, uint8_t* cls) {
+    const SkyProjection S = sky_project_box(P);
+    const SkyTouched T = S.valid ? sky_touched_tiles(P, L) : SkyTouched{};
+    for (int32_t i = 0; i < n; ++i) {
+        const int32_t t = tiles[i];
+        if (sky_tile_clear(S, P.u.resolution[0], P.u.resolution[1], t)) cls[i] = kSkyClear;
+        else cls[i] = (T.valid && t >= 0 && (size_t)t < T.tile.size() && !T.tile[(size_t)t] && sky_tile_crossed(S, P.u.resolution[0], P.u.resolution[1], t)) ? kSkySeeThrough : kSkyMarch;
+    }
+}
+
+inline void sky_split_tiles3(const SceneParams& P, const SkyLiveCells& L, const std::vector<int32_t>& ids, int32_t n_tiles, std::vector<int32_t>& march,
+                             std::vector<int32_t>& clear, std::vector<int32_t>& see) {
+    march.clear(); clear.clear(); see.clear();
+    const int32_t n = ids.empty() ? n_tiles : (int32_t)ids.size();
+    std::vector<int32_t> all;
+    if (ids.empty()) { all.resize((size_t)n); for (int32_t i = 0; i < n; ++i) all[(size_t)i] = i; }
+    const int32_t* t = ids.empty() ? all.data() : ids.data();
+    std::vector<uint8_t> cls((size_t)n);
+    sky_classify_tiles3(P, L, t, n, cls.data());
+    for (int32_t i = 0; i < n; ++i) (cls[(size_t)i] == kSkyClear ? clear : cls[(size_t)i] == kSkySeeThrough ? see : march).push_back(t[i]);
+}
+
+}
diff --git a/volren_amd/csrc/vr_trace.h b/volren_amd/csrc/vr_trace.h
--- a/volren_amd/csrc/vr_trace.h
+++ b/volren_amd/csrc/vr_trace.h
@@ -796,7 +796,7 @@
     h.Tr = 1.0f;
 }
 
-VR_HD bool sky_sample(const SceneParams& P, int32_t px, int32_t py, uint32_t seed, float out[4]) {
+VR_HD bool sky_sample(const SceneParams& P, int32_t px, int32_t py, uint32_t seed, float out[4], bool box_test = true) {
     const int32_t W = P.u.resolution[0], H = P.u.resolution[1];
     const float jx = rng(seed), jy = rng(seed);
     const float fx = (((float)px + jx) - (float)W * 0.5f) / (float)H;
@@ -804,7 +804,7 @@
     const v3 dir = normalize(mat3_mul(P.u.cam_transform, normalize(v3{ fx, fy, P.cam_z })));
     const v3 pos = v3{ P.u.cam_pos[0], P.u.cam_pos[1], P.u.cam_pos[2] };
     float tnear, tfar;
-    if (intersect_box(pos, dir, P.u.vol_bb_min, P.u.vol_bb_max, tnear, tfar)) return false;
+    if (box_test && intersect_box(pos, dir, P.u.vol_bb_min, P.u.vol_bb_max, tnear, tfar)) return false;
     v3 L = v3{ 0.0f, 0.0f, 0.0f };
     if (P.u.show_environment > 0) L = L + (v3{ 1.0f, 1.0f, 1.0f } * 1.0f) * lookup_environment(P, dir);
     out[0] = L.x; out[1] = L.y; out[2] = L.z; out[3] = 0.0f;
diff --git a/volren_amd/renderer.py b/volren_amd/renderer.py
--- a/volren_amd/renderer.py
+++ b/volren_amd/renderer.py
@@ -7,8 +7,8 @@
 _INT_FIELDS = ("sample", "sppx", "seed", "bounces", "show_environment", "tonemapping", "integrator", "grid_frame_counter",
                "sample_pool_mb", "gpu_encoder", "fast_math", "tf_float_atlas", "launch_target_ms", "order_tiles", "coalesce_trace", "majorant_layout",
                "variance", "denoise_iterations", "denoise_moments", "denoise_resolve", "denoise_layers", "denoise_filter", "wide_addressing", "seed_table_mb", "seed_table_max_samples",
-               "expected_skip", "expected_stats", "sky_tiles")
-_READ_ONLY_INT_FIELDS = ("n_grid_frames", "last_launches", "last_sky_tiles", "pending_samples", "majorant_blocked", "env_div_safe", "env_compact", "kernel_variant", "kernel_variant_reason",
+               "expected_skip", "expected_stats", "sky_tiles", "see_through_tiles")
+_READ_ONLY_INT_FIELDS = ("n_grid_frames", "last_launches", "last_sky_tiles", "last_see_through_tiles", "pending_samples", "majorant_blocked", "env_div_safe", "env_compact", "kernel_variant", "kernel_variant_reason",
                          "kernel_wide", "adaptive_rounds", "seed_table_samples", "seed_table_fills")
 _FLOAT_FIELDS = {"tonemap_exposure": 1, "tonemap_gamma": 1, "albedo": 3, "phase": 1, "density_scale": 1,
                  "emission_scale": 1, "vol_clip_min": 3, "vol_clip_max": 3, "env_strength": 1, "env_transform": 9,
```

New measurement: 6150 Msamples/s, median of 6. 5.0% higher.
